# SreenivasVRao/SuperSloMo-VideoInterpolation-PyTorch

Hardware: AMD Instinct MI355X
Metric: interpolated 1280x720 frames/sec (higher is better)
Workload: dtype f32

## Files before the change

include/ssm_hip.h:

```cpp
#ifndef SSM_HIP_H
#define SSM_HIP_H

#include <stddef.h>

#ifdef __cplusplus
extern "C" {
#endif

#define SSM_PADX 4
#define SSM_PADY 3
#define SSM_TAIL_SLACK_FLOATS (1 << 16)

#define SSM_OK 0
#define SSM_E_ARG (-1)
#define SSM_E_LAUNCH (-2)
#define SSM_E_UNSUPPORTED (-3)

#define SSM_FLAG_LRELU 1
#define SSM_FLAG_FP16_FAST 2
#define SSM_FLAG_Q8 4
#define SSM_FLAG_MASK 8

typedef struct ssm_view {
    float *ptr;
    long long sb, sc;
    int sh;
} ssm_view;

typedef struct ssm_hview {
    void *ptr;
    long long sb, sg, sp;
    int sh;
} ssm_hview;

int ssm_abi_version(void);
const char *ssm_last_error_string(void);

void ssm_plane_dims(int H, int W, int *Hp, int *Wp);

int ssm_copy_view(ssm_view src, ssm_view dst, int B, int C, int H, int W, void *stream);

int ssm_conv_config(int k, int Cout, int B, int H, int W, int pool, int *BN, int *CK);
int ssm_conv_plan(int k, int Cin, int Cout, int B, int H, int W, int pool, int ups, int *kind, int *BN, int *CK);
int ssm_conv_force_kind(int kind);

size_t ssm_packed_weight_floats(int Cout, int Cin_padded, int k, int BN);
size_t ssm_packed_bias_floats(int Cout, int BN);

int ssm_pack_weights(const float *w_oihw, const float *bias, float *w_packed, float *bias_packed,
                     int Cout, int Cin, int Cin_padded, int k, int BN, void *stream);

int ssm_conv2d_fwd(ssm_view x1, int C1, ssm_view x2, int C2, const float *w_packed,
                   const float *bias_packed, ssm_view y, ssm_view pool, int B, int H, int W,
                   int Cout, int k, float slope, int flags, void *stream);

int ssm_conv2d_ups_fwd(ssm_view a, int C1, ssm_view b, int C2, const float *w_packed, const float *bias_packed,
                       ssm_view y, int B, int H, int W, int Cout, float slope, int flags, void *stream);

int ssm_conv2d_add_fwd(ssm_view x1, int C1, ssm_view x2, int C2, const float *w_packed, const float *bias_packed, ssm_view y,
                       ssm_view pool, ssm_view add, int add_div, int B, int H, int W, int Cout, int k, float slope, int flags,
                       void *stream);
int ssm_conv2d_ups_add_fwd(ssm_view a, int C1, ssm_view b, int C2, const float *w_packed, const float *bias_packed, ssm_view y,
                           ssm_view add, int add_div, int B, int H, int W, int Cout, float slope, int flags, void *stream);

int ssm_wino_plan(int Cin, int Cout, int B, int H, int W, int ups, int *kind, int *BN, int *CK);
int ssm_wino_force_kind(int kind);
size_t ssm_wino_packed_weight_floats(int Cout, int Cin, int BN);
int ssm_wino_pack_weights(const float *w_oihw, const float *bias, float *w_packed, float *bias_packed, int Cout, int Cin,
                          int BN, void *stream);
int ssm_wino_conv2d_fwd(ssm_view x1, int C1, ssm_view x2, int C2, const float *w_packed, const float *bias_packed,
                        ssm_view y, ssm_view pool, int B, int H, int W, int Cout, float slope, int flags, void *stream);
int ssm_wino_conv2d_ups_fwd(ssm_view a, int C1, ssm_view b, int C2, const float *w_packed, const float *bias_packed,
                            ssm_view y, int B, int H, int W, int Cout, float slope, int flags, void *stream);

int ssm_wino_splitk_plan(int Cin, int Cout, int B, int H, int W, int ups, int BN, int *KS);
int ssm_wino_conv2d_splitk_fwd(ssm_view x1, int C1, ssm_view x2, int C2, const float *w_packed, const float *bias_packed, ssm_view part,
                               int KS, int ups, int B, int H, int W, int Cout, int BN, void *stream);
int ssm_splitk_finish_fwd(ssm_view part, int KS, ssm_view y, ssm_view pool, ssm_view add, int add_div, int B, int C, int H, int W,
                          float slope, int flags, void *stream);
int ssm_conv_splitk_plan(int k, int Cin, int Cout, int B, int H, int W, int *KS);
int ssm_splitk_enable(int wino, int conv);
int ssm_conv2d_splitk_fwd(ssm_view x1, int C1, ssm_view x2, int C2, const float *w_packed, const float *bias_packed, ssm_view part,
                          int KS, int B, int H, int W, int Cout, int k, void *stream);
int ssm_wino_conv2d_add_fwd(ssm_view x1, int C1, ssm_view x2, int C2, const float *w_packed, const float *bias_packed, ssm_view y,
                            ssm_view pool, ssm_view add, int add_div, int B, int H, int W, int Cout, float slope, int flags,
                            void *stream);
int ssm_wino_conv2d_ups_add_fwd(ssm_view a, int C1, ssm_view b, int C2, const float *w_packed, const float *bias_packed, ssm_view y,
                                ssm_view add, int add_div, int B, int H, int W, int Cout, float slope, int flags, void *stream);

int ssm_wino4_plan(int Cin, int Cout, int B, int H, int W, int ups, int *kind, int *BN, int *CK);
int ssm_wino4_preferred(int Cin, int Cout, int B, int H, int W, int ups);
double ssm_wino_estimate(int Cin, int Cout, int B, int H, int W, int ups);
int ssm_wino4_force_kind(int kind);
size_t ssm_wino4_packed_weight_floats(int Cout, int Cin);
int ssm_wino4_pack_weights(const float *w_oihw, const float *bias, float *w_packed, float *bias_packed, int Cout, int Cin, void *stream);
int ssm_wino4_conv2d_add_fwd(ssm_view x1, int C1, ssm_view x2, int C2, const float *w_packed, const float *bias_packed, ssm_view y,
                             ssm_view pool, ssm_view add, int add_div, int B, int H, int W, int Cout, float slope, int flags,
                             void *stream);
int ssm_wino4_conv2d_ups_add_fwd(ssm_view a, int C1, ssm_view b, int C2, const float *w_packed, const float *bias_packed, ssm_view y,
                                 ssm_view add, int add_div, int B, int H, int W, int Cout, float slope, int flags, void *stream);
#define SSM_WINO4_BORDER_TH 16
#define SSM_WINO4_BORDER_TW 32
int ssm_wino4_conv2d_shuffle_fwd(ssm_view x1, int C1, ssm_view x2, int C2, const float *w_packed, const float *bias_packed, ssm_view y, int B,
                                 int H, int W, int Cout4, float slope, int flags, void *stream);
int ssm_wino4_conv2d_ups_border_fwd(ssm_view a, int C1, ssm_view b, int C2, const float *w_packed, const float *bias_packed, ssm_view y, int B,
                                    int H, int W, int Cout, float slope, int flags, void *stream);

int ssm_upgemm_supported(int Cin, int Cout, int H, int W, int k);
int ssm_upgemm_preferred(int Cin, int Cout, int B, int h, int w);
int ssm_upgemm_force_kind(int kind);
size_t ssm_upgemm_packed_weight_floats(int Cout, int Cin);
int ssm_upgemm_pack_weights(const float *w_oihw, float *w_packed, int Cout, int Cin, void *stream);
size_t ssm_upgemm_scratch_floats(int Cout, int B, int h, int w);
int ssm_upgemm_conv2d_ups_add_fwd(ssm_view a, int C1, ssm_view b, int C2, const float *w_packed, const float *bias, ssm_view scratch, ssm_view y,
                                  ssm_view add, int add_div, int B, int H, int W, int Cout, float slope, int flags, void *stream);

int ssm_wino1d_plan(int k, int Cin, int Cout, int B, int H, int W, int *kind, int *BN, int *CK);
int ssm_wino1d_force_kind(int kind);
size_t ssm_wino1d_packed_weight_floats(int Cout, int CinP, int k, int BN);
int ssm_wino1d_pack_weights(const float *w_oihw, const float *bias, float *w_packed, float *bias_packed, int Cout, int Cin,
                            int CinP, int k, int BN, void *stream);
int ssm_wino1d_conv2d_add_fwd(ssm_view x, int Cin, const float *w_packed, const float *bias_packed, ssm_view y, ssm_view pool,
                              ssm_view add, int add_div, int B, int H, int W, int Cout, int k, float slope, int flags, void *stream);

int ssm_wino7_plan(int Cin, int Cout, int B, int H, int W, int *kind);
int ssm_wino7_force_kind(int kind);
size_t ssm_wino7_packed_weight_floats(int Cout, int Cin);
int ssm_wino7_pack_weights(const float *w_oihw, const float *bias, float *w_packed, float *bias_packed, int Cout, int Cin, void *stream);
int ssm_wino7_conv2d_add_fwd(ssm_view x, int Cin, const float *w_packed, const float *bias_packed, ssm_view y, ssm_view pool,
                             ssm_view add, int add_div, int B, int H, int W, int Cout, float slope, int flags, void *stream);

int ssm_wino5_plan(int Cin, int Cout, int B, int H, int W, int *kind);
int ssm_wino5_force_kind(int kind);
size_t ssm_wino5_packed_weight_floats(int Cout, int CinP);
int ssm_wino5_pack_weights(const float *w_oihw, const float *bias, float *w_packed, float *bias_packed, int Cout, int Cin, int CinP,
                           void *stream);
int ssm_wino5_conv2d_add_fwd(ssm_view x, int Cin, const float *w_packed, const float *bias_packed, ssm_view y, ssm_view pool,
                             ssm_view add, int add_div, int B, int H, int W, int Cout, float slope, int flags, void *stream);

enum { SSM_PACK_DIRECT = 0, SSM_PACK_WINO = 1, SSM_PACK_WINO1D = 2, SSM_PACK_WINO4 = 3, SSM_PACK_WINO7 = 4, SSM_PACK_WINO5 = 5 };
typedef struct {
    const float *w;
    const float *bias;
    float *wp, *bp;
    int Cout, Cin, CinP, k, BN, algo, transposed, nbias;
    long long first, total;
} ssm_pack32_job;
int ssm_pack32_weights_batch(const ssm_pack32_job *jobs_device, int n_jobs, long long total_elements, void *stream);
int ssm_pack32_wino_tiles_batch(const ssm_pack32_job *jobs_device, int n_jobs, long long total_tiles, int max_bn, void *stream);

int ssm_conv16_config(int k, int Cout, int W, int *BN, int *KYS);
int ssm_conv16_plan(int k, int Cin, int Cout, int W, int ups, int flags, int *kind, int *BN, int *KYS);
size_t ssm_packed16_weight_halves(int Cout, int Cin_padded, int k, int BN);
int ssm_pack16_weights(const float *w_oihw, const float *bias, void *w_packed, float *bias_packed, int Cout,
                       int Cin, int Cin_padded, int k, int BN, int KYS, float scale, void *stream);
int ssm_conv2d_hl8_fwd(ssm_hview x1, int C1, ssm_hview x2, int C2, const void *w_packed,
                       const float *bias_packed, float wscale, ssm_hview y_hl8, ssm_view y_f32,
                       ssm_hview pool_hl8, int B, int H, int W, int Cout, int k, float slope, int flags,
                       void *stream);
int ssm_conv16_ups_config(int Cout, int W, int *BN, int *KYS);
int ssm_conv2d_ups_hl8_fwd(ssm_hview a, int C1, ssm_hview b, int C2, const void *w_packed,
                           const float *bias_packed, float wscale, ssm_hview y_hl8, ssm_view y_f32, int B, int H,
                           int W, int Cout, float slope, int flags, void *stream);
int ssm_conv16q_config(int k, int Cout, int W, int *BN, int *KYS);
int ssm_conv16q_ups_config(int Cout, int W, int *BN, int *KYS);
size_t ssm_packed16q_weight_bytes(int Cout, int Cin_padded, int k, int BN, int KYS);
int ssm_pack16q_weights(const float *w_oihw, const float *bias, void *w_packed, float *bias_packed, int Cout, int Cin,
                        int Cin_padded, int k, int BN, int KYS, float scale, void *stream);
int ssm_flowinterp_inputs_hq8_fwd(ssm_view img6, ssm_view flow4, const float *t, ssm_hview out16, ssm_view flows4, int B, int H,
                                  int W, void *stream);
int ssm_conv2d_hl8_subpixel_fwd(ssm_hview x1, int C1, ssm_hview x2, int C2, const void *w_packed, const float *bias_packed,
                                float inv_wscale, ssm_hview y_hl8, int B, int H, int W, int Cr, int transposed, float slope, int flags,
                                void *stream);
typedef struct ssm_subpixel_problem {
    ssm_hview x1;
    int C1;
    ssm_hview x2;
    int C2;
    const void *w_packed;
    const float *bias_packed;
    float inv_wscale;
    ssm_hview y_hl8;
    int H, W;
    int transposed;
    int skip_y, skip_x;
} ssm_subpixel_problem;
size_t ssm_conv16_subpixel_table_bytes(int n);
int ssm_conv16_subpixel_plan(const ssm_subpixel_problem *problems, int n, int B, int Cr, int wcfg, float slope, int flags,
                             void *table_host, size_t table_bytes, int *block_start);
int ssm_conv16_subpixel_run(const void *table_device, int n, const int *block_start, int Cr, int wcfg, int Cin, void *stream);
int ssm_hl8_gather_cols(ssm_hview a, int Ga, ssm_hview b, int Gb, ssm_hview dst, int B, int H, int col0, int ncols, int col1,
                        void *stream);
typedef struct ssm_pack16q_job {
    const float *w;
    const float *bias;
    void *wp;
    float *bp;
    int Cout, Cin, CinP, k, BN, KYS;
    float scale;
    int transposed;
    int block_start, row_blocks;
} ssm_pack16q_job;
int ssm_pack16q_job_blocks(int Cout, int CinP, int k, int BN, int *row_blocks, int *bias_blocks);
int ssm_pack16q_weights_batch(const ssm_pack16q_job *jobs_device, int n_jobs, int total_blocks, void *stream);
int ssm_hq8_from_f32(ssm_view src, ssm_hview dst, int B, int C, int G, int H, int W, void *stream);
int ssm_hq8_to_f32(ssm_hview src, ssm_view dst, int B, int C, int G, int H, int W, void *stream);
int ssm_hl8_from_f32(ssm_view src, ssm_hview dst, int B, int C, int G, int H, int W, void *stream);
int ssm_hl8_to_f32(ssm_hview src, ssm_view dst, int B, int C, int G, int H, int W, void *stream);

int ssm_upsample2x_cat_hl8_fwd(ssm_hview a, int Ga, ssm_hview b, int Gb, ssm_hview y, int B, int h, int w,
                               void *stream);
int ssm_flowinterp_inputs_hl8_fwd(ssm_view img6, ssm_view flow4, const float *t, ssm_hview out16,
                                  ssm_view flows4, int B, int H, int W, void *stream);

int ssm_avgpool2_fwd(ssm_view x, ssm_view y, int B, int C, int H, int W, void *stream);

int ssm_upsample2x_cat_fwd(ssm_view a, int Ca, ssm_view b, int Cb, ssm_view y, int B, int h, int w,
                           void *stream);

int ssm_warp_bilinear_fwd(ssm_view img, ssm_view flow, ssm_view out, int B, int C, int H, int W,
                          void *stream);

int ssm_flowinterp_inputs_fwd(ssm_view img6, ssm_view flow4, const float *t, ssm_view out16, int B,
                              int H, int W, void *stream);
int ssm_flowinterp_inputs_t_fwd(ssm_view img6, ssm_view flow4, const float *t, ssm_view out16, int B, int H, int W, void *stream);

int ssm_synthesize_fwd(ssm_view img6, ssm_view in16, ssm_view out5, const float *t, ssm_view y3,
                       ssm_view aux, int B, int H, int W, void *stream);

int ssm_synthesize_upscaled_fwd(ssm_view img6, ssm_view aux_lo, const float *t, ssm_view y3, int B, int H, int W, int s, void *stream);

int ssm_tile_stitch_fwd(ssm_view tile, ssm_view out, int N, int C, int window_h, int window_w, int Hp, int Wp, int oy, int ox, int cy0,
                        int cx0, int cy1, int cx1, int seams, int b, void *stream);

int ssm_final_conv_fwd(ssm_view x, const float *w_oihw, const float *bias, int NC, ssm_view out, ssm_view img6, ssm_view in16,
                       const float *t, ssm_view y3, ssm_view aux, int B, int H, int W, void *stream);

int ssm_program_create(void **handle);
int ssm_program_destroy(void *handle);
int ssm_program_begin(void *handle, void *const *streams, int n_streams);
int ssm_program_mark(void *handle, int *n_nodes);
int ssm_program_end(void *handle, int *n_nodes);
int ssm_program_run(void *handle, int first, int last, void *const *streams, int n_streams);
int ssm_stream_wait(void *src_stream, void *dst_stream);

int ssm_frames_from_u8_fwd(const unsigned char *frames_hwc, ssm_view out, int N, int H, int W, int Hp, int Wp,
                           int top, int left, const float *mean3, const float *std3, int pad_before_norm,
                           void *stream);
int ssm_frames_to_u8_fwd(ssm_view in, unsigned char *frames_hwc, int N, int H, int W, int top, int left,
                         const float *mean3, const float *std3, int mode, void *stream);

#define SSM_YUV_ROW 20
#define SSM_YUV_BT601 0
#define SSM_YUV_BT709 1
#define SSM_YUV_LIMITED 0
#define SSM_YUV_FULL 1
#define SSM_YUV_420_CENTRED 0
#define SSM_YUV_420_COSITED 1
#define SSM_YUV_444 2
// ... 154 lines not shown
```

superslomo-videointerpolation-pytorch_amd/csrc/ssm_wino4.hip:

```cpp
#include "ssm_conv_host.h"
#include "ssm_device.h"

#include <atomic>
#include <mutex>
#include <type_traits>
#include <cstdlib>

namespace {

struct W4Params {
    const float *src1;
    const float *src2;
    long long sb1, sb2;
    long long sc;
    int sh;
    int C1, Cin;
    const float *wpk;
    const float *bias;
    float *dst;
    long long dsb, dsc;
    int dsh;
    float *pool;
    long long psb, psc;
    int psh;
    int H, W, Cout;
    int hs, ws;
    int tilesX, tilesY, NB;
    float slope;
    int lrelu;
    int vec;
    int abl;
    unsigned long long *dbg;
    int trace_block;
    int stagger;
    int border;
    const float *add;
    long long asb, asc;
    int ash, adiv;
};

template <int GTX_, int WTY_, int WTX_, int NCB_ = 1>
struct W4Cfg {
    static constexpr int GTX = GTX_, GTY = 16 / GTX_, WTY = WTY_, WTX = WTX_, NCB = NCB_;
    static constexpr int NW = 4 * NCB, THREADS = 64 * NW;
    static constexpr int CK = 4, BN = 32 * NCB, NT = 32;
    static constexpr int NTX = GTX * WTX, NTY = GTY * WTY;
    static constexpr int TH = 4 * NTY, TW = 4 * NTX;
    static constexpr int PH = TH + 2, PW = TW + 8, PW4 = PW / 4;
    static constexpr int SHIFT = 1;
    static constexpr int USZ1 = CK * 9 * 32 * 4, USZ = NCB * USZ1;
    static constexpr int PSZ = CK * PH * PW;
    static constexpr int VSZ = CK * 9 * NT * 4;
    static constexpr int LH = TH / 2 + 2, LW = TW / 2 + 8, LW4 = LW / 4;
    static constexpr int RSZ = CK * LH * LW;
    static constexpr int NPOS = (TH / 2 + 1) * (TW / 2 + 1);
    static_assert(WTY * WTX == 2 && (GTX == 4 || GTX == 8 || GTX == 16) && (NCB == 1 || NCB == 2), "two tile groups of 16 tiles");
    static_assert(USZ1 % 256 == 0 && NPOS <= 256, "filter stage = whole 1-KiB DMA groups; expander: one position per thread");
};

template <class C, bool UPS>
struct W4Lds {
    static constexpr int DSZ = UPS ? C::RSZ : C::PSZ;
    static constexpr int DH = UPS ? C::LH : C::PH, DW4 = UPS ? C::LW4 : C::PW4;
    static constexpr int NGU = C::USZ / 256;
    static constexpr int NDQ = DSZ / 4;
    static constexpr int NGP = (NDQ + 63) / 64;
    static constexpr int NW = C::NCB == 2 ? 4 : C::NW;
    static constexpr int NIU = (NGU + NW - 1) / NW, NIP = (NGP + NW - 1) / NW, NI = NIU + NIP;
    static constexpr int NBUF = C::NCB == 2 ? 2 : 1;
    static constexpr int UOFF = 0;
    static constexpr int DOFF = 2 * C::USZ;
    static constexpr int DCAP = NGP * 256 + 256;
    static constexpr int NBD = 2;
    static constexpr int HOFF = DOFF + NBD * DCAP;
    static constexpr int HCAP = C::PSZ + 4;
    static constexpr int POFF = UPS ? HOFF : DOFF;
    static constexpr int PCAP = UPS ? HCAP : DCAP;
    static constexpr int VOFF = HOFF + (UPS ? NBUF * HCAP : 0);
    static constexpr int BYTES = (VOFF + NBUF * C::VSZ) * 4;
    static_assert(VOFF % 4 == 0 && DOFF % 4 == 0 && HOFF % 4 == 0 && HCAP % 4 == 0 && DCAP % 4 == 0, "16-byte aligned regions");
    static_assert(BYTES + (C::NCB == 2 ? 256 : 0) <= (C::NCB == 1 ? 80 : 160) * 1024, "LDS budget (two workgroups of 256 or one of 512 per CU; 64-cout form: + its biases)");
};

#define W4_PA 0.625
#define W4_PB 1.6
constexpr float kA = (float)W4_PA, kB = (float)W4_PB, kA2 = (float)(W4_PA * W4_PA), kB2 = (float)(W4_PB * W4_PB);
constexpr float kA3 = (float)(W4_PA * W4_PA * W4_PA), kB3 = (float)(W4_PB * W4_PB * W4_PB);
constexpr float kP0 = (float)(W4_PA * W4_PA * W4_PB * W4_PB), kS2 = (float)(W4_PA * W4_PA + W4_PB * W4_PB);

__host__ __device__ constexpr int w4_freq(int i, int j) { return 18 * (j / 3) + 3 * i + (j % 3); }

__device__ __forceinline__ void w4_row_pass(int hh, const float *d, float *x) {
    if (hh == 0) {
        const float te = d[4] - kB2 * d[2], to = d[3] - kB2 * d[1];
        x[0] = (kP0 * d[0] - kS2 * d[2]) + d[4];
        x[1] = te + kA * to;
        x[2] = te - kA * to;
    } else {
        const float ue = d[4] - kA2 * d[2], uo = d[3] - kA2 * d[1];
        x[0] = ue + kB * uo;
        x[1] = ue - kB * uo;
        x[2] = (kP0 * d[1] - kS2 * d[3]) + d[5];
    }
}

__device__ __forceinline__ void w4_col_pass(float x0, float x1, float x2, float x3, float x4, float x5, float *v, int stride) {
    const float te = x4 - kB2 * x2, to = x3 - kB2 * x1;
    const float ue = x4 - kA2 * x2, uo = x3 - kA2 * x1;
    v[0] = (kP0 * x0 - kS2 * x2) + x4;
    v[stride] = te + kA * to;
    v[2 * stride] = te - kA * to;
    v[3 * stride] = ue + kB * uo;
    v[4 * stride] = ue - kB * uo;
    v[5 * stride] = (kP0 * x1 - kS2 * x3) + x5;
}

__device__ __forceinline__ void w4_col_pass_half(int hq, float x0, float x1, float x2, float x3, float x4, float x5, float *v, int stride) {
    if (hq == 0) {
        const float te = x4 - kB2 * x2, to = x3 - kB2 * x1;
        v[0] = (kP0 * x0 - kS2 * x2) + x4;
        v[stride] = te + kA * to;
        v[2 * stride] = te - kA * to;
    } else {
        const float ue = x4 - kA2 * x2, uo = x3 - kA2 * x1;
        v[0] = ue + kB * uo;
        v[stride] = ue - kB * uo;
        v[2 * stride] = (kP0 * x1 - kS2 * x3) + x5;
    }
}

template <int NT>
__device__ __forceinline__ void w4_store_v9(int part, const float *v, f32x4 *vo) {
    float *vf = (float *)vo;
    if (part == 0) {
        vo[0] = f32x4{v[0], v[1], v[2], v[3]};
        vo[NT] = f32x4{v[4], v[5], v[6], v[7]};
        vf[2 * NT * 4] = v[8];
    } else if (part == 1) {
        vf[2 * NT * 4 + 1] = v[0];
        *(f32x2 *)(vf + 2 * NT * 4 + 2) = f32x2{v[1], v[2]};
        vo[3 * NT] = f32x4{v[3], v[4], v[5], v[6]};
        *(f32x2 *)(vf + 4 * NT * 4) = f32x2{v[7], v[8]};
    } else if (part == 2) {
        *(f32x2 *)(vf + 4 * NT * 4 + 2) = f32x2{v[0], v[1]};
        vo[5 * NT] = f32x4{v[2], v[3], v[4], v[5]};
        *(f32x2 *)(vf + 6 * NT * 4) = f32x2{v[6], v[7]};
        vf[6 * NT * 4 + 2] = v[8];
    } else {
        vf[6 * NT * 4 + 3] = v[0];
        vo[7 * NT] = f32x4{v[1], v[2], v[3], v[4]};
        vo[8 * NT] = f32x4{v[5], v[6], v[7], v[8]};
    }
}

template <int NT>
__device__ __forceinline__ void w4_store_v(int hh, const float *v, f32x4 *vo) {
    if (hh == 0) {
#pragma unroll
        for (int g = 0; g < 4; ++g) vo[g * NT] = f32x4{v[4 * g], v[4 * g + 1], v[4 * g + 2], v[4 * g + 3]};
        *(f32x2 *)(vo + 4 * NT) = f32x2{v[16], v[17]};
    } else {
        *((f32x2 *)(vo + 4 * NT) + 1) = f32x2{v[0], v[1]};
#pragma unroll
        for (int g = 0; g < 4; ++g) vo[(5 + g) * NT] = f32x4{v[2 + 4 * g], v[3 + 4 * g], v[4 + 4 * g], v[5 + 4 * g]};
    }
}

#ifdef SSM_WINO_ABLATE
#define W4ABL(bit) (p.abl & (bit))
#elif defined(W4_CT_ABL)
#define W4ABL(bit) (W4_CT_ABL & (bit))
#else
#define W4ABL(bit) 0
#endif

template <bool SHUF>
__device__ __forceinline__ void w4_epilogue_shuffle(const W4Params &p, const f32x4 (&acc)[36], const float (&bv)[4], int b, int cu0, int q, int px, int py);

__device__ __forceinline__ void w4_epilogue(const W4Params &p, const f32x4 (&acc)[36], const float (&bv)[4], int b, int cu0, int q, int px, int py) {
        const float sl = (p.lrelu & 1) ? p.slope : 1.f;
        const bool amask = (p.lrelu & 2) != 0;
        float *dstb = p.dst + (long long)b * p.dsb;
        float *poolb = p.pool ? p.pool + (long long)b * p.psb : nullptr;
                const unsigned pb = 4u * ((unsigned)(4 * q) * (unsigned)p.dsc + (unsigned)py * (unsigned)p.dsh + (unsigned)px);
        const unsigned qb = 4u * ((unsigned)(4 * q) * (unsigned)p.psc + (unsigned)(py >> 1) * (unsigned)p.psh + (unsigned)(px >> 1));
        const bool vok = py + 4 <= p.H && px + 4 <= p.W && p.vec;
        const float *addb = p.add ? p.add + (long long)(b / p.adiv) * p.asb + (long long)(4 * q) * p.asc + (long long)py * p.ash + px : nullptr;
#pragma unroll
        for (int r = 0; r < 4; ++r) {
            const int cu = cu0 + r;
            float t[4][6];
#pragma unroll
            for (int j = 0; j < 6; ++j) {
                const float m0 = acc[w4_freq(0, j)][r], m1 = acc[w4_freq(1, j)][r], m2 = acc[w4_freq(2, j)][r], m3 = acc[w4_freq(3, j)][r],
                            m4 = acc[w4_freq(4, j)][r], m5 = acc[w4_freq(5, j)][r];
                const float s1 = m1 + m2, d1 = m1 - m2, s2 = m3 + m4, d2 = m3 - m4;
                t[0][j] = (m0 + s1) + s2;
                t[1][j] = kA * d1 + kB * d2;
                t[2][j] = kA2 * s1 + kB2 * s2;
                t[3][j] = (kA3 * d1 + m5) + kB3 * d2;
            }
            float y[4][4];
#pragma unroll
            for (int i = 0; i < 4; ++i) {
                const float s1 = t[i][1] + t[i][2], d1 = t[i][1] - t[i][2], s2 = t[i][3] + t[i][4], d2 = t[i][3] - t[i][4];
                y[i][0] = ((t[i][0] + s1) + s2) + bv[r];
                y[i][1] = (kA * d1 + kB * d2) + bv[r];
                y[i][2] = (kA2 * s1 + kB2 * s2) + bv[r];
                y[i][3] = ((kA3 * d1 + t[i][5]) + kB3 * d2) + bv[r];
            }
            if (addb) {
                const float *ap = addb + (long long)cu * p.asc;
#pragma unroll
                for (int i = 0; i < 4; ++i) {
                    if (vok) {
                        const f32x4 z = *(const f32x4 *)(ap + (long long)i * p.ash);
                        if (amask) {
#pragma unroll
                            for (int e = 0; e < 4; ++e) y[i][e] *= z[e] > 0.f ? 1.f : p.slope;
                        } else {
                            y[i][0] += z[0];
                            y[i][1] += z[1];
                            y[i][2] += z[2];
                            y[i][3] += z[3];
                        }
                    } else {
#pragma unroll
                        for (int e = 0; e < 4; ++e)
                            if (py + i < p.H && px + e < p.W) {
                                const float z = ap[(long long)i * p.ash + e];
                                if (amask) y[i][e] *= z > 0.f ? 1.f : p.slope;
                                else y[i][e] += z;
                            }
                    }
                }
            }
#pragma unroll
            for (int i = 0; i < 4; ++i)
#pragma unroll
                for (int e = 0; e < 4; ++e) y[i][e] = fmaxf(y[i][e], y[i][e] * sl);
            float *bp = dstb + (long long)cu * p.dsc;
#pragma unroll
            for (int i = 0; i < 4; ++i) {
                if (vok) {
                    store_sbase(bp + (long long)i * p.dsh, pb, f32x4{y[i][0], y[i][1], y[i][2], y[i][3]});
                } else {
#pragma unroll
                    for (int e = 0; e < 4; ++e)
                        if (py + i < p.H && px + e < p.W) store_sbase(bp + (long long)i * p.dsh + e, pb, y[i][e]);
                }
            }
            if (poolb) {
                float *qp = poolb + (long long)cu * p.psc;
#pragma unroll
                for (int i = 0; i < 2; ++i) {
                    const float o0 = ((y[2 * i][0] + y[2 * i + 1][0]) + (y[2 * i][1] + y[2 * i + 1][1])) * 0.25f;
                    const float o1 = ((y[2 * i][2] + y[2 * i + 1][2]) + (y[2 * i][3] + y[2 * i + 1][3])) * 0.25f;
                    const bool rok = py + 2 * i < p.H;
                    if (rok && px + 4 <= p.W && p.vec) store_sbase(qp + (long long)i * p.psh, qb, f32x2{o0, o1});
                    else if (rok) {
                        if (px + 2 <= p.W) store_sbase(qp + (long long)i * p.psh, qb, o0);
                        if (px + 4 <= p.W) store_sbase(qp + (long long)i * p.psh + 1, qb, o1);
                    }
                }
            }
            __builtin_amdgcn_sched_barrier(0);
        }
}

__device__ __forceinline__ void w4_output_tile(const f32x4 (&acc)[36], int r, float bias, float sl, float (&y)[4][4]) {
    float t[4][6];
#pragma unroll
    for (int j = 0; j < 6; ++j) {
        const float m0 = acc[w4_freq(0, j)][r], m1 = acc[w4_freq(1, j)][r], m2 = acc[w4_freq(2, j)][r], m3 = acc[w4_freq(3, j)][r],
                    m4 = acc[w4_freq(4, j)][r], m5 = acc[w4_freq(5, j)][r];
        const float s1 = m1 + m2, d1 = m1 - m2, s2 = m3 + m4, d2 = m3 - m4;
        t[0][j] = (m0 + s1) + s2;
        t[1][j] = kA * d1 + kB * d2;
        t[2][j] = kA2 * s1 + kB2 * s2;
        t[3][j] = (kA3 * d1 + m5) + kB3 * d2;
    }
#pragma unroll
    for (int i = 0; i < 4; ++i) {
        const float s1 = t[i][1] + t[i][2], d1 = t[i][1] - t[i][2], s2 = t[i][3] + t[i][4], d2 = t[i][3] - t[i][4];
        y[i][0] = ((t[i][0] + s1) + s2) + bias;
        y[i][1] = (kA * d1 + kB * d2) + bias;
        y[i][2] = (kA2 * s1 + kB2 * s2) + bias;
        y[i][3] = ((kA3 * d1 + t[i][5]) + kB3 * d2) + bias;
    }
#pragma unroll
    for (int i = 0; i < 4; ++i)
#pragma unroll
        for (int e = 0; e < 4; ++e) y[i][e] = fmaxf(y[i][e], y[i][e] * sl);
}

template <>
__device__ __forceinline__ void w4_epilogue_shuffle<true>(const W4Params &p, const f32x4 (&acc)[36], const float (&bv)[4], int b, int cu0, int q, int px, int py) {
    const float sl = (p.lrelu & 1) ? p.slope : 1.f;
    float *dstb = p.dst + (long long)b * p.dsb + (long long)(cu0 >> 2) * p.dsc;
    const unsigned pb = 4u * ((unsigned)q * (unsigned)p.dsc + (unsigned)(2 * py) * (unsigned)p.dsh + (unsigned)(2 * px));
    const bool vok = py + 4 <= p.H && px + 4 <= p.W && p.vec;
#pragma unroll
    for (int a = 0; a < 2; ++a) {
        float y0[4][4], y1[4][4];
        w4_output_tile(acc, 2 * a, bv[2 * a], sl, y0);
        w4_output_tile(acc, 2 * a + 1, bv[2 * a + 1], sl, y1);
#pragma unroll
        for (int i = 0; i < 4; ++i) {
            const float *rowp = dstb + (long long)(2 * i + a) * p.dsh;
            if (vok) {
                store_sbase_nop(rowp, pb, f32x4{y0[i][0], y1[i][0], y0[i][1], y1[i][1]});
                store_sbase_nop(rowp + 4, pb, f32x4{y0[i][2], y1[i][2], y0[i][3], y1[i][3]});
            } else {
#pragma unroll
                for (int e = 0; e < 4; ++e) {
                    if (py + i < p.H && px + e < p.W) {
                        store_sbase(rowp + 2 * e, pb, y0[i][e]);
                        store_sbase(rowp + 2 * e + 1, pb, y1[i][e]);
                    }
                }
            }
        }
        __builtin_amdgcn_sched_barrier(0);
    }
}

template <class C, bool UPS, bool SHUF = false>
__global__ __launch_bounds__(C::THREADS, 2) void wino4_kernel(const W4Params p) {
    extern __shared__ __attribute__((aligned(16))) float lds[];
    using L = W4Lds<C, UPS>;
    constexpr int BN = C::BN, PH = C::PH, PW = C::PW, CK = C::CK, NT = C::NT, NW = C::NW, NCB = C::NCB;

    const int tid = threadIdx.x;
    const int lane = tid & 63, l15 = lane & 15, q = lane >> 4;
    const int wid = __builtin_amdgcn_readfirstlane(tid >> 6);
    const int cb = wid & 1, tg = (wid >> 1) & 1, blk = wid >> 2;

    int id = ssm_xcd_tile(blockIdx.x, gridDim.x);
    const int nb = id % p.NB;
    id /= p.NB;
    int tx, ty, b;
    if (UPS && C::NCB == 1 && p.border) {
        const int nbt = 2 * p.tilesX + 2 * (p.tilesY - 2);
        const int k = id % nbt;
        b = id / nbt;
        if (k < 2 * p.tilesX) {
            ty = k < p.tilesX ? 0 : p.tilesY - 1;
            tx = k < p.tilesX ? k : k - p.tilesX;
        } else {
            const int kk = k - 2 * p.tilesX;
            ty = 1 + (kk >> 1);
            tx = (kk & 1) ? p.tilesX - 1 : 0;
        }
    } else {
        tx = id % p.tilesX;
        id /= p.tilesX;
        ty = id % p.tilesY;
        b = id / p.tilesY;
    }
    const int x0 = tx * C::TW, y0 = ty * C::TH;

    const long long porg = UPS ? (long long)(y0 / 2 - 1) * p.sh + (x0 / 2 - 4) : (long long)(y0 - 1) * p.sh + (x0 - 4);
    const float *pbase1 = p.src1 + (long long)b * p.sb1 + porg;
    const float *pbase2 = p.src2 + (long long)b * p.sb2 + porg;
    const float *wbase = p.wpk + (long long)nb * NCB * p.Cin * (9 * 32 * 4);

    int poff[L::NIP];
#pragma unroll
    for (int i = 0; i < L::NIP; ++i) {
        const int qq = (i * L::NW + (wid & (L::NW - 1))) * 64 + lane;
        if (qq < L::NDQ) {
            const int c = qq / (L::DH * L::DW4);
            const int rem = qq - c * (L::DH * L::DW4);
            const int r = rem / L::DW4;
            const int j = rem - r * L::DW4;
            const int sH = UPS ? p.hs : p.H, sW = UPS ? p.ws : p.W, sy = UPS ? y0 / 2 - 1 : y0 - 1, sx = UPS ? x0 / 2 : x0;
            const int re = min(r, sH + (SSM_PADY - 1) - sy), fe = min(4 * j, ((sW + 2 * SSM_PADX + 3) & ~3) - 4 - sx);
            poff[i] = ((int)(c * p.sc) + re * p.sh + fe) * 4;
        } else {
            poff[i] = 0;
        }
    }
    const int uoff = lane * 16;
    int uoffk[L::NIU];
#pragma unroll
    for (int k = 0; k < L::NIU; ++k) uoffk[k] = lane * 16 + k * (L::NW * 1024);
    const unsigned lds0 = (unsigned)(size_t)(__attribute__((address_space(3))) void *)lds;

    auto issue_k = [&](int ch, int stage, int k, int pbuf = 0) {
        constexpr int NW = L::NW;
        if (NCB == 2 && wid >= NW) return;
        const int c0 = ch * CK;
        if (k < L::NIU) {
            const int g = NW * k + wid;
            if (NW * k + NW - 1 < L::NGU || g < L::NGU) {
                constexpr int G1 = C::USZ1 / 256;
                const int gb = NCB == 1 ? 0 : g / G1;
                const float *base = wbase + ((long long)gb * p.Cin + c0) * (9 * 32 * 4) + (g - gb * G1) * 256;
                const unsigned m0v = __builtin_amdgcn_readfirstlane(lds0 + (unsigned)(L::UOFF + stage * C::USZ) * 4u + (unsigned)g * 1024u);
                lds_dma16(base, uoff, m0v);
            }
        } else {
            const int kk = k - L::NIU;
            const int g = NW * kk + wid;
            if (NW * kk + NW - 1 < L::NGP || g < L::NGP) {
                const float *base = (c0 < p.C1) ? pbase1 + (long long)c0 * p.sc : pbase2 + (long long)(c0 - p.C1) * p.sc;
                const unsigned m0v = __builtin_amdgcn_readfirstlane(lds0 + (unsigned)(L::DOFF + pbuf * L::DCAP) * 4u + (unsigned)g * 1024u + (UPS ? 0u : 4u * C::SHIFT));
                lds_dma16(base, poff[kk], m0v);
            }
        }
    };

    f32x4 acc[36];
#pragma unroll
    for (int f = 0; f < 36; ++f) acc[f] = f32x4{0.f, 0.f, 0.f, 0.f};

    const int nchunks = p.Cin / CK;
    if (p.stagger > 0 && ((blockIdx.x >> 8) & 1)) {
        for (int i = 0; i < p.stagger; ++i) __builtin_amdgcn_s_sleep(1);
    }
    static_assert(L::NI <= (NCB == 2 ? 18 : 9), "DMA issue slots of the matrix loop: one per frequency group (two in the 512-thread form)");
    auto issue_n = [&](int ch, int stage, int n) { issue_k(ch, stage, n < L::NIP ? L::NIU + n : n - L::NIP); };
    const bool u_full = wid < L::NGU - NW * (L::NIU - 1);
    if constexpr (NCB == 1) {
#pragma unroll
        for (int n = 0; n < L::NI; ++n) issue_n(0, 0, n);
        if (p.Cin / CK > 1) {
#pragma unroll
            for (int k = L::NIU; k < L::NI; ++k) issue_k(1, 0, k, 1);
        }
    }
    float bv[4];
    if constexpr (NCB == 2) {
        if (tid < BN) lds[L::BYTES / 4 + tid] = p.bias[nb * BN + tid];
    } else {
#pragma unroll
        for (int r = 0; r < 4; ++r) bv[r] = p.bias[nb * BN + blk * 32 + cb * 16 + 4 * q + r];
    }

    const int thh = (wid >> 1) & 1;
    const int thq = wid >> 2;
    const int tu = tid & 127;
    const int tcin = tu >> 5, ttile = tu & 31;
    const int tgx = (ttile & 15) % C::GTX, tgy = (ttile & 15) / C::GTX, tg2 = ttile >> 4;
    const int tTx = (tg2 % C::WTX) * C::GTX + tgx, tTy = (tg2 / C::WTX) * C::GTY + tgy;
    const int t_src = L::POFF + (UPS ? 0 : C::SHIFT) + (tcin * PH + 4 * tTy) * PW + 4 * tTx + 3 + (UPS ? C::SHIFT : 0);
    const int t_dst = L::VOFF / 4 + (tcin * 9) * NT + ttile;

    const f32x4 *lds4 = (const f32x4 *)lds;
    const int aBase = L::UOFF / 4 + blk * (C::USZ1 / 4) + q * (9 * 32) + cb * 16 + l15;
    const int bBase = L::VOFF / 4 + q * (9 * NT) + tg * 16 + l15;

    int ex_r0 = 0, ex_r1 = 0, ex_dd = 0, ex_fl = 0;
    if constexpr (UPS) {
        constexpr int PRW = C::TW / 2 + 1, NPOS = C::NPOS, LW = C::LW;
        const int etid = threadIdx.x & 255;
        const int ly0 = y0 / 2 - 1, lx0 = x0 / 2 - 1;
        const int pi = etid / PRW, pj = etid - pi * PRW;
        const int i = ly0 + pi, j = lx0 + pj;
        const int i0 = min(max(i, 0), p.hs - 1), i1 = min(max(i + 1, 0), p.hs - 1);
        const int j0 = min(max(j, 0), p.ws - 1), j1 = min(max(j + 1, 0), p.ws - 1);
        const int Y = 2 * i + 1, X = 2 * j + 1;
        const bool yt = Y >= 0 && Y < p.H, yb2 = Y + 1 < p.H, xl = X >= 0 && X < p.W, xr = X + 1 < p.W;
        ex_fl = (j0 == j1 ? 1 : 0) | (i0 == i1 ? 2 : 0) | ((yt && xl) ? 4 : 0) | ((yt && xr) ? 8 : 0) | ((yb2 && xl) ? 16 : 0) | ((yb2 && xr) ? 32 : 0) |
                (etid < NPOS ? 64 : 0);
        ex_r0 = (i0 - ly0) * LW + 3 - lx0 + j0;
        ex_r1 = (i1 - ly0) * LW + 3 - lx0 + j0;
        ex_dd = (2 * pi) * PW + 2 * pj + 3 + C::SHIFT;
    }
    auto expand = [&](int rbuf, int hbuf, auto CB, auto CN) {
        if constexpr (UPS) {
            constexpr int LH = C::LH, LW = C::LW;
            constexpr int cbeg = decltype(CB)::value, cnum = decltype(CN)::value;
            const float *raw = lds + L::DOFF + rbuf * L::DCAP + cbeg * LH * LW;
            float *hip = lds + L::HOFF + hbuf * L::HCAP + cbeg * PH * PW;
            if (ex_fl & 64) {
                const bool jeq = ex_fl & 1, ieq = ex_fl & 2;
                const float ex_xa = jeq ? 1.f : 0.75f, ex_xb = jeq ? 0.f : 0.25f;
                const float ex_ca = jeq ? 1.f : 0.25f, ex_cw = jeq ? 0.f : 0.75f;
                const float ya = ieq ? 1.f : 0.75f, yb = ieq ? 0.f : 0.25f;
                const float ex_a00 = (ex_fl & 4) ? ya : 0.f, ex_b00 = (ex_fl & 4) ? yb : 0.f;
                const float ex_a01 = (ex_fl & 8) ? ya : 0.f, ex_b01 = (ex_fl & 8) ? yb : 0.f;
                const float ex_a10 = (ex_fl & 16) ? yb : 0.f, ex_b10 = (ex_fl & 16) ? ya : 0.f;
                const float ex_a11 = (ex_fl & 32) ? yb : 0.f, ex_b11 = (ex_fl & 32) ? ya : 0.f;
                const float *r0 = raw + ex_r0, *r1 = raw + ex_r1;
                float *dd = hip + ex_dd;
                float v00[cnum], v01[cnum], v10[cnum], v11[cnum];
#pragma unroll
                for (int cc = 0; cc < cnum; ++cc) {
                    v00[cc] = r0[cc * LH * LW];
                    v01[cc] = r0[cc * LH * LW + 1];
                    v10[cc] = r1[cc * LH * LW];
                    v11[cc] = r1[cc * LH * LW + 1];
                }
#pragma unroll
                for (int cc = 0; cc < cnum; ++cc) {
                    const float h00 = ex_xa * v00[cc] + ex_xb * v01[cc], h01 = ex_ca * v00[cc] + ex_cw * v01[cc];
                    const float h10 = ex_xa * v10[cc] + ex_xb * v11[cc], h11 = ex_ca * v10[cc] + ex_cw * v11[cc];
                    dd[cc * PH * PW] = ex_a00 * h00 + ex_b00 * h10;
                    dd[cc * PH * PW + 1] = ex_a01 * h01 + ex_b01 * h11;
                    dd[cc * PH * PW + PW] = ex_a10 * h00 + ex_b10 * h10;
                    dd[cc * PH * PW + PW + 1] = ex_a11 * h01 + ex_b11 * h11;
                }
            }
        }
    };

    auto transform_as = [&](auto HH, auto HQ, int sbuf, int vbuf) {
        constexpr int hh = decltype(HH)::value, hq = decltype(HQ)::value;
        const float *rp = lds + t_src + sbuf * L::PCAP;
        f32x4 *vo = (f32x4 *)lds + t_dst + vbuf * (C::VSZ / 4);
        f32x4 a4[6];
        f32x2 a2[6];
#pragma unroll
        for (int i = 0; i < 6; ++i) {
            a4[i] = *(const f32x4 *)(rp + i * PW);
            a2[i] = *(const f32x2 *)(rp + i * PW + 4);
        }
        float X[6][3];
#pragma unroll
        for (int i = 0; i < 6; ++i) {
            const float d[6] = {a4[i][0], a4[i][1], a4[i][2], a4[i][3], a2[i][0], a2[i][1]};
            w4_row_pass(hh, d, X[i]);
        }
        if constexpr (NCB == 1) {
            float v[18];
#pragma unroll
            for (int jj = 0; jj < 3; ++jj) w4_col_pass(X[0][jj], X[1][jj], X[2][jj], X[3][jj], X[4][jj], X[5][jj], v + jj, 3);
            w4_store_v<NT>(hh, v, vo);
        } else {
            float v[9];
#pragma unroll
            for (int jj = 0; jj < 3; ++jj) w4_col_pass_half(hq, X[0][jj], X[1][jj], X[2][jj], X[3][jj], X[4][jj], X[5][jj], v + jj, 3);
            w4_store_v9<NT>(2 * hh + hq, v, vo);
        }
    };
    auto transform = [&](int sbuf = 0, int vbuf = 0) {
        using I0 = std::integral_constant<int, 0>;
        using I1 = std::integral_constant<int, 1>;
        if constexpr (NCB == 1) {
            if (thh == 0) transform_as(I0{}, I0{}, sbuf, vbuf);
            else transform_as(I1{}, I0{}, sbuf, vbuf);
        } else {
            if (thh == 0) {
                if (thq == 0) transform_as(I0{}, I0{}, sbuf, vbuf);
                else transform_as(I0{}, I1{}, sbuf, vbuf);
            } else {
                if (thq == 0) transform_as(I1{}, I0{}, sbuf, vbuf);
                else transform_as(I1{}, I1{}, sbuf, vbuf);
            }
        }
    };

#ifdef SSM_WINO_ABLATE
    unsigned long long tph[5] = {0, 0, 0, 0, 0};
    const bool stamp = (p.abl & 32) && p.dbg;
    unsigned long long tk = stamp ? __builtin_amdgcn_s_memtime() : 0;
    const unsigned long long tstart = tk;
#define W4STAMP(i)                                              \
    if (stamp) {                                                \
        const unsigned long long tn = __builtin_amdgcn_s_memtime(); \
        tph[i] += tn - tk;                                      \
        tk = tn;                                                \
    }
    const bool trace = (p.abl & 128) && p.dbg && blockIdx.x == 0;
#define W4TRACE(chv, pt)                                                                                             \
    if (trace && (chv) < 16 && lane == 0) p.dbg[16 + (wid * 16 + (chv)) * 4 + (pt)] = __builtin_amdgcn_s_memtime();
#elif defined(W4_TRACE)
#define W4STAMP(i)
    unsigned long long *ltrace = (unsigned long long *)(lds + L::BYTES / 4 + 64);
    const bool trace = p.dbg && blockIdx.x == (unsigned)p.trace_block;
#define W4TRACE(chv, pt) \
    if (trace && (chv) < 16 && lane == 0) ltrace[(wid * 16 + (chv)) * 4 + (pt)] = __builtin_amdgcn_s_memtime();
    if (trace && lane == 0) ltrace[(wid * 16 + 0) * 4 + 1] = __builtin_amdgcn_s_memtime();
#else
#define W4STAMP(i)
#define W4TRACE(chv, pt)
#endif
    f32x4 a[3], bq[3];
    auto matrix = [&](int stage, int vbuf, auto dma, auto slot) __attribute__((always_inline)) {
        const int ai = aBase + stage * (C::USZ / 4), bi = bBase + vbuf * (C::VSZ / 4);
        a[0] = lds4[ai];
        bq[0] = lds4[bi];
        a[1] = lds4[ai + 32];
        bq[1] = lds4[bi + NT];
#pragma unroll
        for (int g = 0; g < 9; ++g) {
            const int cur = g % 3, nxt = (g + 2) % 3;
#pragma unroll
            for (int e = 0; e < 4; ++e) {
                acc[4 * g + e] = __builtin_amdgcn_mfma_f32_16x16x4f32(a[cur][e], bq[cur][e], acc[4 * g + e], 0, 0, 0);
                if (e == 0) {
                    __builtin_amdgcn_sched_barrier(0);
                    if (g + 2 < 9 && !W4ABL(8)) {
                        a[nxt] = lds4[ai + (g + 2) * 32];
                        bq[nxt] = lds4[bi + (g + 2) * NT];
                    }
                    __builtin_amdgcn_sched_barrier(0);
                }
                if constexpr (NCB == 2) {
                    slot(4 * g + e);
                    __builtin_amdgcn_sched_barrier(0);
                }
                if constexpr (NCB == 2) {
                    if ((e == 1 || e == 3) && 2 * g + (e == 3) < L::NI) {
                        dma(2 * g + (e == 3));
                        __builtin_amdgcn_sched_barrier(0);
                    }
                } else if (e == 1 && g < L::NI) {
                    dma(g);
                    __builtin_amdgcn_sched_barrier(0);
                }
            }
            __builtin_amdgcn_sched_barrier(0);
        }
    };

    if constexpr (NCB == 1) {
        static_assert(L::NGP % L::NW == 0, "every wave brings NIP patch pieces per chunk");
        auto chunk1 = [&](int ch, auto N1, auto N2) __attribute__((always_inline)) {
            constexpr bool n1 = decltype(N1)::value, n2 = decltype(N2)::value;
            const int stage = ch & 1;
            if (u_full) wait_vmcnt<L::NIU + (n1 ? L::NIP : 0)>();
            else wait_vmcnt<L::NIU - 1 + (n1 ? L::NIP : 0)>();
            __syncthreads();
            W4STAMP(0)
            if constexpr (UPS) {
                expand(stage, 0, std::integral_constant<int, 0>{}, std::integral_constant<int, CK>{});
                __syncthreads();
            }
            if (!W4ABL(4) || ch == 0) transform(UPS ? 0 : stage, 0);
            W4STAMP(1)
            wait_vmcnt<n1 ? L::NIP : 0>();
            __syncthreads();
            W4STAMP(2)
            const int (&uk)[L::NIU] = uoffk;
            const int (&pk)[L::NIP] = poff;
            const int c1 = (ch + 1) * CK, c2 = (ch + 2) * CK;
            const float *fb = wbase + wid * 256 + (long long)c1 * (9 * 32 * 4);
            const float *pb = (c2 < p.C1) ? pbase1 + (long long)c2 * p.sc : pbase2 + (long long)(c2 - p.C1) * p.sc;
            const unsigned mu = __builtin_amdgcn_readfirstlane(lds0 + (unsigned)(L::UOFF + (stage ^ 1) * C::USZ) * 4u + (unsigned)wid * 1024u);
            const unsigned mp = __builtin_amdgcn_readfirstlane(lds0 + (unsigned)(L::DOFF + stage * L::DCAP) * 4u + (unsigned)wid * 1024u + (UPS ? 0u : 4u * C::SHIFT));
            matrix(stage, 0, [&](int n) {
                if (W4ABL(1) && ch >= 1) return;
                constexpr int NW = L::NW;
                if (n < L::NIU) {
                    if constexpr (n1) {
                        if (NW * n + NW - 1 < L::NGU || NW * n + wid < L::NGU)
                            lds_dma16(fb, uk[n], mu + (unsigned)(n * NW * 1024));
                    }
                } else if constexpr (n2) {
                    const int k = n - L::NIU;
                    lds_dma16(pb, pk[k], mp + (unsigned)(k * NW * 1024));
                }
            }, [](int) {});
            W4STAMP(3)
        };
        using T = std::true_type;
        using F = std::false_type;
        int ch = 0;
        for (; ch + 2 < nchunks; ++ch) chunk1(ch, T{}, T{});
        if (ch + 1 < nchunks) chunk1(ch++, T{}, F{});
        chunk1(ch, F{}, F{});

    } else {
        using T = std::true_type;
        using F = std::false_type;
#pragma unroll
        for (int k = 0; k < L::NI; ++k) issue_k(0, 0, k, 0);
        if (nchunks > 1) {
#pragma unroll
            for (int k = L::NIU; k < L::NI; ++k) issue_k(1, 0, k, 1);
        }
        wait_vmcnt<0>();
        __syncthreads();
        using C0 = std::integral_constant<int, 0>;
        using C2 = std::integral_constant<int, 2>;
        auto expand_half = [&](int rbuf, int hbuf) {
            if (blk == 0) expand(rbuf, hbuf, C0{}, C2{});
            else expand(rbuf, hbuf, C2{}, C2{});
        };
        if constexpr (UPS) {
            expand_half(0, 0);
            if (nchunks > 1) expand_half(1, 1);
            __syncthreads();
            if (nchunks > 2) {
#pragma unroll
                for (int k = L::NIU; k < L::NI; ++k) issue_k(2, 0, k, 0);
            }
        }
        transform(0, 0);
        f32x4 r4[6];
        f32x2 r2[6];
        float tX[6][3];
        float tv18[18];
        auto tstep2 = [&](auto HH, int m, const float *src, f32x4 *vo) __attribute__((always_inline)) {
            constexpr int hh = decltype(HH)::value;
            if (m < 6) {
                r4[m] = *(const f32x4 *)(src + m * PW);
                r2[m] = *(const f32x2 *)(src + m * PW + 4);
            }
            if (m >= 3 && m < 9) {
                const int i = m - 3;
                const float d[6] = {r4[i][0], r4[i][1], r4[i][2], r4[i][3], r2[i][0], r2[i][1]};
                w4_row_pass(hh, d, tX[i]);
            }
            if (m >= 9 && m < 18) {
                const int jj = (m - 9) / 3, st3 = (m - 9) % 3;
                const float x0v = tX[0][jj], x1v = tX[1][jj], x2v = tX[2][jj], x3v = tX[3][jj], x4v = tX[4][jj], x5v = tX[5][jj];
                if (st3 == 0) {
                    tv18[jj] = (kP0 * x0v - kS2 * x2v) + x4v;
                    tv18[15 + jj] = (kP0 * x1v - kS2 * x3v) + x5v;
                }
                if (st3 == 1) {
                    const float te = x4v - kB2 * x2v, to = x3v - kB2 * x1v;
                    tv18[3 + jj] = te + kA * to;
                    tv18[6 + jj] = te - kA * to;
                }
                if (st3 == 2) {
                    const float ue = x4v - kA2 * x2v, uo = x3v - kA2 * x1v;
                    tv18[9 + jj] = ue + kB * uo;
                    tv18[12 + jj] = ue - kB * uo;
                }
            }
            if (m >= 18 && m < 23) {
                const int k = m - 18;
                if (hh == 0) {
                    if (k < 4) vo[k * NT] = f32x4{tv18[4 * k], tv18[4 * k + 1], tv18[4 * k + 2], tv18[4 * k + 3]};
                    else *(f32x2 *)(vo + 4 * NT) = f32x2{tv18[16], tv18[17]};
                } else {
                    if (k == 0) *((f32x2 *)(vo + 4 * NT) + 1) = f32x2{tv18[0], tv18[1]};
                    else vo[(4 + k) * NT] = f32x4{tv18[4 * k - 2], tv18[4 * k - 1], tv18[4 * k], tv18[4 * k + 1]};
                }
            }
        };
        auto chunk = [&](int ch, auto STEADY, auto HH, auto HQ) __attribute__((always_inline)) {
            constexpr bool steady = decltype(STEADY)::value;
            const bool m1 = steady || ch + 1 < nchunks, m2 = steady || ch + 2 < nchunks, m3 = steady || ch + 3 < nchunks;
            const int st = ch & 1;
            wait_vmcnt<0>();
            if (!W4ABL(16) || ch == 0) __syncthreads();
            W4STAMP(0)
            W4TRACE(ch, 0)
            const float *tsrc = lds + t_src + (st ^ 1) * L::PCAP;
            f32x4 *tdst = (f32x4 *)lds + t_dst + (st ^ 1) * (C::VSZ / 4);
            matrix(st, st, [&](int g) {
                if (W4ABL(1) || decltype(HQ)::value != 0) return;
                if (g < L::NIU) {
                    if (m1) issue_k(ch + 1, st ^ 1, g, 0);
                } else if constexpr (UPS) {
                    if (m3) issue_k(ch + 3, 0, g, st ^ 1);
                } else {
                    if (m2) issue_k(ch + 2, 0, g, st);
                }
            }, [&](int m) {
                if constexpr (decltype(HQ)::value == 1) {
                    if (m1 && !W4ABL(4)) tstep2(HH, m, tsrc, tdst);
                }
            });
            W4STAMP(3)
            W4TRACE(ch, 2)
            if constexpr (UPS) {
                if (m2 && decltype(HQ)::value == 0) expand(st, st, C0{}, std::integral_constant<int, CK>{});
            }
            W4STAMP(1)
            W4TRACE(ch, 3)
        };
        auto chunks = [&](auto HH, auto HQ) __attribute__((always_inline)) {
            if constexpr (decltype(HQ)::value == 1) __builtin_amdgcn_s_setprio(1);
            int ch = 0;
            for (; ch + 3 < nchunks; ++ch) chunk(ch, T{}, HH, HQ);
            for (; ch < nchunks; ++ch) chunk(ch, F{}, HH, HQ);
        };
        using I0 = std::integral_constant<int, 0>;
        using I1 = std::integral_constant<int, 1>;
        if (thh == 0) {
            if (thq == 0) chunks(I0{}, I0{});
            else chunks(I0{}, I1{});
        } else {
            if (thq == 0) chunks(I1{}, I0{});
            else chunks(I1{}, I1{});
        }
    }

#if defined(SSM_WINO_ABLATE) || defined(W4_CT_ABL)
    if (W4ABL(2) && acc[0][0] != 12345.678f) return;
#endif
    {
        if constexpr (NCB == 2) {
            const f32x4 b4 = *(const f32x4 *)(lds + L::BYTES / 4 + blk * 32 + cb * 16 + 4 * q);
            bv[0] = b4[0], bv[1] = b4[1], bv[2] = b4[2], bv[3] = b4[3];
        }
        const int gx = l15 % C::GTX, gy = l15 / C::GTX;
        const int Tx = (tg % C::WTX) * C::GTX + gx, Ty = (tg / C::WTX) * C::GTY + gy;
        if constexpr (SHUF) w4_epilogue_shuffle<true>(p, acc, bv, b, nb * BN + blk * 32 + cb * 16, q, x0 + 4 * Tx, y0 + 4 * Ty);
        else w4_epilogue(p, acc, bv, b, nb * BN + blk * 32 + cb * 16, q, x0 + 4 * Tx, y0 + 4 * Ty);
    }
#if defined(W4_TRACE) && !defined(SSM_WINO_ABLATE)
    if (trace) {
        if (lane == 0) ltrace[(wid * 16 + 1) * 4 + 1] = __builtin_amdgcn_s_memtime();
        wait_vmcnt<0>();
        if (lane == 0) ltrace[(wid * 16 + 2) * 4 + 1] = __builtin_amdgcn_s_memtime();
        __syncthreads();
        for (int i = tid; i < NW * 64; i += C::THREADS) p.dbg[16 + i] = ltrace[i];
    }
#endif
#ifdef SSM_WINO_ABLATE
    if (stamp) {
        wait_vmcnt<0>();
        W4STAMP(4)
        if (tid == 0) {
            for (int i = 0; i < 5; ++i) atomicAdd(p.dbg + i, tph[i]);
            atomicAdd(p.dbg + 5, tk - tstart);
            atomicAdd(p.dbg + 6, 1ULL);
        }
    }
#endif
}

using X4A = W4Cfg<8, 2, 1>;
using X4B = W4Cfg<16, 2, 1>;
using X4C = W4Cfg<4, 1, 2>;

using Y4A = W4Cfg<8, 2, 1, 2>;
using Y4B = W4Cfg<16, 2, 1, 2>;
using Y4C = W4Cfg<4, 1, 2, 2>;


#define SSM_W4_KINDS(X) X(X4A_, X4A) X(X4B_, X4B) X(X4C_, X4C) X(Y4A_, Y4A) X(Y4B_, Y4B) X(Y4C_, Y4C)

enum W4Kind {
#define X(name, cfg) name,
    SSM_W4_KINDS(X)
#undef X
        NW4KIND
};

struct W4KindInfo {
    int th, tw, bn;
};

constexpr W4KindInfo kW4Info[NW4KIND] = {
#define X(name, cfg) W4KindInfo{cfg::TH, cfg::TW, cfg::BN},
    SSM_W4_KINDS(X)
#undef X
};

ssm::ForcedKind g_force_w4kind;
constexpr ssm::OutRules kW4Rules = { true,  4,  false};
#if defined(SSM_WINO_ABLATE) || defined(W4_TRACE)
std::atomic<unsigned long long *> g_w4dbg{nullptr};
#endif

double estimate_w4(const W4KindInfo &ki, int Cin, int Cout, int B, int H, int W, int ups) {
    const long long tiles = (long long)B * ((W + ki.tw - 1) / ki.tw) * ((H + ki.th - 1) / ki.th);
    const long long nwg = tiles * (Cout / ki.bn);
    const double chunks = (double)Cin / 4.0;
    if (ki.bn == 64) {
        const double per = chunks * 3500.0 + 24000.0;
        return (double)((nwg + 255) / 256) * per;
    }
    const double per = chunks * (4500.0 + (ups ? 250.0 : 0.0)) + 11000.0;
    const long long full = nwg / 512, rem = nwg % 512;
    double t = (double)full * per;
    if (rem) t += rem > 256 ? per : chunks * (3300.0 + (ups ? 250.0 : 0.0)) + 11000.0;
    return t;
}

int pick_w4kind(int Cin, int Cout, int B, int H, int W, int ups) {
    const int forced = g_force_w4kind.get(NW4KIND);
    if (forced >= 0) return forced;
    int best = -1;
    double bt = 0.0;
    static const int allow_wide = [] {
        const char *e = getenv("SSM_WINO4_WIDE");
        return e ? atoi(e) : 1;
    }();
    for (int i = 0; i < NW4KIND; ++i) {
        if (kW4Info[i].bn == 64 && (!allow_wide || Cout % 64)) continue;
        const double t = estimate_w4(kW4Info[i], Cin, Cout, B, H, W, ups);
        if (best < 0 || t < bt * 0.999) {
            best = i;
            bt = t;
        }
    }
    return best;
}

template <class C, bool UPS, bool SHUF = false>
int w4launch(W4Params &p, int B, hipStream_t st) {
    p.tilesX = (p.W + C::TW - 1) / C::TW;
    p.tilesY = (p.H + C::TH - 1) / C::TH;
    if (p.Cout % C::BN) {
        ssm::set_error("wino4 conv: tile configuration of %d couts per workgroup, Cout = %d", C::BN, p.Cout);
        return SSM_E_UNSUPPORTED;
    }
    p.NB = p.Cout / C::BN;
    if (p.border && (!UPS || p.tilesX < 2 || p.tilesY < 2)) {
        ssm::set_error("wino4 conv: a border-ring launch needs the fused-upsample form and at least 2 x 2 workgroup tiles (%d x %d)", p.tilesX, p.tilesY);
        return SSM_E_UNSUPPORTED;
    }
    const long long ntiles = p.border ? 2LL * p.tilesX + 2LL * (p.tilesY - 2) : (long long)p.tilesX * p.tilesY;
    const long long blocks = ntiles * p.NB * B;
    int lds_bytes = W4Lds<C, UPS>::BYTES + (C::NCB == 2 ? C::BN * 4 : 0);
#ifdef W4_TRACE
    lds_bytes += 4096;
#endif
#ifdef SSM_WINO_ABLATE
    if (const char *e = getenv("SSM_WINO4_SOLO"))
        if (atoi(e) && lds_bytes < 100 * 1024) lds_bytes = 100 * 1024;
#endif
    return ssm::launch_tiles<wino4_kernel<C, UPS, SHUF>>("wino4 conv", UPS ? "ssm_wino4_conv2d_ups_fwd" : "ssm_wino4_conv2d_fwd", blocks, C::THREADS,
                                                          lds_bytes, st, p);
}

template <bool UPS>
int w4dispatch(int kind, W4Params &p, int B, hipStream_t st) {
    switch (kind) {
#define X(name, cfg) \
    case name: return w4launch<cfg, UPS>(p, B, st);
        SSM_W4_KINDS(X)
#undef X
    }
    ssm::set_error("wino4 conv: tile configuration %d is not available for this problem", kind);
    return SSM_E_UNSUPPORTED;
}

__global__ void wino4_pack_kernel(const float *__restrict__ w, const float *__restrict__ bias, float *__restrict__ wp,
                                  float *__restrict__ bp, int Cout, int Cin, long long total, int nbias) {
    const long long idx = (long long)blockIdx.x * blockDim.x + threadIdx.x;
    if (idx < total) {
        long long r = idx;
        const int e = (int)(r % 4);
        r /= 4;
        const int n = (int)(r % 32);
        r /= 32;
        const int fq = (int)(r % 9);
        r /= 9;
        const int cin = (int)(r % Cin);
        const int nb = (int)(r / Cin);
        const int co = nb * 32 + n, f = 4 * fq + e, i = (f % 18) / 3, j = 3 * (f / 18) + f % 3;
        double val = 0.0;
        if (co < Cout) {
            auto grow = [](int f, double (&g)[3]) {
                const double p = f == 0 ? 0.0 : f == 1 ? W4_PA : f == 2 ? -W4_PA : f == 3 ? W4_PB : -W4_PB;
                if (f == 5) {
                    g[0] = g[1] = 0.0;
                    g[2] = 1.0;
                    return;
                }
                double nrm = 1.0;
#pragma unroll
                for (int o = 0; o < 5; ++o) {
                    const double po = o == 0 ? 0.0 : o == 1 ? W4_PA : o == 2 ? -W4_PA : o == 3 ? W4_PB : -W4_PB;
                    if (o != f) nrm *= p - po;
                }
                g[0] = 1.0 / nrm;
                g[1] = p / nrm;
                g[2] = p * p / nrm;
            };
            double gi[3], gj[3];
            grow(i, gi);
            grow(j, gj);
            const float *g = w + ((long long)co * Cin + cin) * 9;
#pragma unroll
            for (int a = 0; a < 3; ++a)
#pragma unroll
                for (int c = 0; c < 3; ++c) val += gi[a] * (double)g[3 * a + c] * gj[c];
        }
        wp[idx] = (float)val;
    }
    if (idx < nbias) bp[idx] = (idx < Cout) ? bias[idx] : 0.f;
}

int w4fill(W4Params &p, ssm_view x1, int C1, ssm_view x2, int C2, const float *w_packed, const float *bias_packed, ssm_view y, ssm_view pool,
           ssm_view add, int add_div, int B, int H, int W, int Cout, float slope, int flags, int srcW) {
    SSM_REQUIRE(B > 0 && H > 0 && W > 0 && Cout > 0 && C1 > 0 && C2 >= 0, "wino4 conv: bad sizes");
    SSM_REQUIRE(Cout % 32 == 0, "wino4 conv: Cout (%d) must be a multiple of 32", Cout);
    SSM_REQUIRE(x1.ptr && y.ptr && w_packed && bias_packed, "wino4 conv: null pointer");
    SSM_REQUIRE(C1 % 4 == 0 && C2 % 4 == 0, "wino4 conv: channel counts (%d,%d) must be multiples of 4", C1, C2);
    SSM_TRY(ssm::check_source("wino4 conv", true, x1, srcW, w_packed));
    SSM_TRY(ssm::check_source2("wino4 conv", x1, x2, C2));
    SSM_REQUIRE(4LL * x1.sc * 4 < 0x7fffffffLL, "wino4 conv: channel stride too large");
    p.src1 = x1.ptr;
    p.src2 = C2 > 0 ? x2.ptr : x1.ptr;
    p.sb1 = x1.sb;
    p.sb2 = C2 > 0 ? x2.sb : 0;
    p.sc = x1.sc;
    p.sh = x1.sh;
    p.C1 = C1;
    p.Cin = C1 + C2;
    p.wpk = w_packed;
    p.bias = bias_packed;
    p.hs = H / 2;
    p.ws = W / 2;
    p.abl = 0;
    p.border = 0;
#ifdef SSM_WINO_ABLATE
    if (const char *e = getenv("SSM_WINO4_ABL")) p.abl = atoi(e);
#endif
#if defined(SSM_WINO_ABLATE) || defined(W4_TRACE)
    p.dbg = g_w4dbg.load();
#else
    p.dbg = nullptr;
#endif
    static const int stagger = [] {
        const char *e = getenv("SSM_WINO4_STAGGER");
        return e ? atoi(e) : 0;
    }();
    p.stagger = stagger;
    p.trace_block = 0;
#ifdef W4_TRACE
    if (const char *e = getenv("SSM_W4_TRACE_BLOCK")) p.trace_block = atoi(e);
#endif
    return ssm::bind_outputs("wino4 conv", kW4Rules, p, y, pool, add, add_div, B, H, W, Cout, slope, flags);
}

}

extern "C" int ssm_wino4_plan(int Cin, int Cout, int B, int H, int W, int ups, int *kind, int *BN, int *CK) {
    if (Cin % 4 || Cout % 32 || Cin <= 0 || Cout <= 0) {
        ssm::set_error("wino4 conv: no tile configuration for Cin=%d Cout=%d (Cin a multiple of 4, Cout a multiple of 32)", Cin, Cout);
        return SSM_E_UNSUPPORTED;
    }
    if (kind) *kind = pick_w4kind(Cin, Cout, B, H, W, ups);
    if (BN) *BN = 32;
    if (CK) *CK = 4;
    return SSM_OK;
}

#if defined(SSM_WINO_ABLATE) || defined(W4_TRACE)
extern "C" int ssm_wino4_debug_buffer(unsigned long long *dev_counters) {
    g_w4dbg.store(dev_counters);
    return SSM_OK;
}
#endif

extern "C" int ssm_wino4_preferred(int Cin, int Cout, int B, int H, int W, int ups) {
    if (Cin % 4 || Cout % 32 || Cin <= 0 || Cout <= 0) return 0;
    if ((long long)H * W < 2048) return 0;
    return 1;
}

extern "C" int ssm_wino4_force_kind(int kind) {
    return g_force_w4kind.set(kind, NW4KIND);
}

extern "C" size_t ssm_wino4_packed_weight_floats(int Cout, int Cin) { return (size_t)(Cout / 32) * (size_t)Cin * 9 * 32 * 4; }

extern "C" int ssm_wino4_pack_weights(const float *w, const float *bias, float *wp, float *bp, int Cout, int Cin, void *stream) {
    SSM_REQUIRE(w && bias && wp && bp, "wino4 pack_weights: null pointer");
    SSM_REQUIRE(Cout > 0 && Cin > 0 && Cout % 32 == 0, "wino4 pack_weights: bad sizes (Cout a multiple of 32)");
    const long long total = (long long)ssm_wino4_packed_weight_floats(Cout, Cin);
    const int nbias = Cout;
    const long long n = total > nbias ? total : nbias;
    SSM_LAUNCH(wino4_pack_kernel, dim3((unsigned)((n + 255) / 256)), dim3(256), 0, (hipStream_t)stream, w, bias, wp, bp, Cout, Cin,
                       total, nbias);
    return ssm::check_launch("ssm_wino4_pack_weights");
}

extern "C" int ssm_wino4_conv2d_add_fwd(ssm_view x1, int C1, ssm_view x2, int C2, const float *w_packed, const float *bias_packed, ssm_view y,
                                        ssm_view pool, ssm_view add, int add_div, int B, int H, int W, int Cout, float slope, int flags,
                                        void *stream) {
    int kind = 0;
    const int rc = ssm_wino4_plan(C1 + C2, Cout, B, H, W, 0, &kind, nullptr, nullptr);
    if (rc != SSM_OK) return rc;
    W4Params p;
    const int rf = w4fill(p, x1, C1, x2, C2, w_packed, bias_packed, y, pool, add, add_div, B, H, W, Cout, slope, flags, W);
    if (rf != SSM_OK) return rf;
    return w4dispatch<false>(kind, p, B, (hipStream_t)stream);
}

extern "C" int ssm_wino4_conv2d_shuffle_fwd(ssm_view x1, int C1, ssm_view x2, int C2, const float *w_packed, const float *bias_packed, ssm_view y,
                                            int B, int H, int W, int Cout4, float slope, int flags, void *stream) {
    SSM_REQUIRE(Cout4 > 0 && Cout4 % 64 == 0, "wino4 conv_shuffle: 4 Cout (%d) must be a multiple of 64", Cout4);
    int kind = 0;
    const int rc = ssm_wino4_plan(C1 + C2, Cout4, B, H, W, 0, &kind, nullptr, nullptr);
    if (rc != SSM_OK) return rc;
    if (kW4Info[kind].bn != 64) kind = Y4A_;
    W4Params p;
    const ssm_view none = {nullptr, 0, 0, 0};
    const int rf = w4fill(p, x1, C1, x2, C2, w_packed, bias_packed, y, none, none, 1, B, H, W, Cout4, slope, flags, W);
    if (rf != SSM_OK) return rf;
    switch (kind) {
        case Y4A_: return w4launch<Y4A, false, true>(p, B, (hipStream_t)stream);
        case Y4B_: return w4launch<Y4B, false, true>(p, B, (hipStream_t)stream);
        default: return w4launch<Y4C, false, true>(p, B, (hipStream_t)stream);
    }
}

extern "C" int ssm_wino4_conv2d_ups_border_fwd(ssm_view a, int C1, ssm_view b, int C2, const float *w_packed, const float *bias_packed, ssm_view y,
                                               int B, int H, int W, int Cout, float slope, int flags, void *stream) {
    SSM_REQUIRE(H % 2 == 0 && W % 2 == 0, "wino4 conv_ups_border: the output of a x2 upsample has even H, W (got %dx%d)", H, W);
    SSM_REQUIRE(C1 + C2 > 0 && (C1 + C2) % 4 == 0 && Cout % 32 == 0, "wino4 conv_ups_border: Cin a multiple of 4, Cout of 32");
    W4Params p;
    const ssm_view none = {nullptr, 0, 0, 0};
    const int rf = w4fill(p, a, C1, b, C2, w_packed, bias_packed, y, none, none, 1, B, H, W, Cout, slope, flags, W / 2);
    if (rf != SSM_OK) return rf;
    p.border = 1;
    return w4launch<X4A, true>(p, B, (hipStream_t)stream);
}

extern "C" int ssm_wino4_conv2d_ups_add_fwd(ssm_view a, int C1, ssm_view b, int C2, const float *w_packed, const float *bias_packed, ssm_view y,
                                            ssm_view add, int add_div, int B, int H, int W, int Cout, float slope, int flags, void *stream) {
    int kind = 0;
    SSM_REQUIRE(H % 2 == 0 && W % 2 == 0, "wino4 conv_ups: the output of a x2 upsample has even H, W (got %dx%d)", H, W);
    const int rc = ssm_wino4_plan(C1 + C2, Cout, B, H, W, 1, &kind, nullptr, nullptr);
    if (rc != SSM_OK) return rc;
    W4Params p;
    const ssm_view none = {nullptr, 0, 0, 0};
    const int rf = w4fill(p, a, C1, b, C2, w_packed, bias_packed, y, none, add, add_div, B, H, W, Cout, slope, flags, W / 2);
    if (rf != SSM_OK) return rf;
    return w4dispatch<true>(kind, p, B, (hipStream_t)stream);
}
```

superslomo-videointerpolation-pytorch_amd/ssm_amd/engine.py:

```python
import os

import torch

from . import hipbind as hb
from .weights import RECURRENT_HIDDEN, RECURRENT_LAYERS, param_key, recurrent_convs, unet_layers


class KernelTimer:

    def __init__(self):
        self.spans = []

    def span(self, family, name, flops=0.0, nbytes=0.0, issued=None):
        e0, e1 = torch.cuda.Event(enable_timing=True), torch.cuda.Event(enable_timing=True)
        self.spans.append((family, name, flops, nbytes, e0, e1, flops if issued is None else issued))
        return e0, e1

    def summary(self):
        out = {}
        for fam, name, fl, nb, e0, e1, isd in self.spans:
            d = out.setdefault(fam, {"ms": 0.0, "flops": 0.0, "issued": 0.0, "bytes": 0.0, "launches": 0, "by_name": {}})
            ms = e0.elapsed_time(e1)
            d["ms"] += ms
            d["flops"] += fl
            d["issued"] += isd
            d["bytes"] += nb
            d["launches"] += 1
            n = d["by_name"].setdefault(name, [0.0, 0.0, 0])
            n[0] += ms
            n[1] += fl
            n[2] += 1
        return out


MODES = ("f32", "f32w", "f16x3", "f16", "f16f8")


def base_mode(mode):
    return "f32" if mode == "f32w" else mode


HOIST_PAIR_PARTS = os.environ.get("SSM_HOIST", "1") != "0"

WINO_SKIP = frozenset(n for n in os.environ.get("SSM_WINO_SKIP", "").split(",") if n)

WINO1D = os.environ.get("SSM_WINO1D", "57")


WINO7 = os.environ.get("SSM_WINO7", "1")
WINO5 = os.environ.get("SSM_WINO5", "1")


WINO4 = os.environ.get("SSM_WINO4", "1")


TRAIN_WINO4 = os.environ.get("SSM_TRAIN_WINO4", "1")
TRAIN_FWD_BLOCKED = os.environ.get("SSM_TRAIN_FWD_BLOCKED", "1")


WINO4_SUBPIXEL = tuple(n for n in os.environ.get("SSM_WINO4_SUBPIXEL", "conv11a").split(",") if n not in ("", "0"))


UPGEMM = os.environ.get("SSM_UPGEMM", "1")


def upgemm_enabled(name):
    return UPGEMM not in ("0", "") and (UPGEMM == "1" or name in UPGEMM.split(","))


def wino4_enabled(name):
    return WINO4 not in ("0", "") and (WINO4 == "1" or name in WINO4.split(","))


def wino1d_enabled(k):
    return k in (5, 7) and str(k) in WINO1D


def choose_algo(name, ci, co, k, nb, h, w, ups, wino, wino1d, wino4=None, blocked2d=None, upgemm=True):
    skip = name in WINO_SKIP or "all" in WINO_SKIP or name == "final_conv"
    wino4 = wino1d if wino4 is None else wino4
    blocked2d = wino1d if blocked2d is None else blocked2d
    if (upgemm and wino and wino1d and ups and not skip and k == 3 and upgemm_enabled(name) and hb.upgemm_supported(ci, co, h, w, k)
            and (UPGEMM != "1" or hb.upgemm_preferred(ci, co, nb, h, w))):
        return "upgemm"
    if blocked2d and not skip and k == 7 and WINO7 not in ("0", "") and hb.wino7_supported(ci, co, h, w, k):
        return "wino7"
    if blocked2d and not skip and k == 5 and WINO5 not in ("0", "") and ci % 4 == 0 and hb.wino5_supported(ci, co, h, w, k):
        return "wino5"
    if wino1d and not skip and wino1d_enabled(k) and hb.wino1d_supported(ci, co, h, w, k):
        return "wino1d"
    if wino and not skip and hb.wino_supported(ci, co, h, w, k):
        if (wino4 and wino4_enabled(name) and hb.wino4_supported(ci, co, h, w, k)
                and (WINO4 != "1" or hb.wino4_preferred(ci, co, nb, h, w, ups))):
            return "wino4"
        return "wino"
    return "direct"


_ALGO_CLASS = {name: (lambda form=form: form.cls) for name, form in hb.FORMS.items()}
ISSUED_FACTOR = {name: form.issued for name, form in hb.FORMS.items()}


def issued_factor(pk):
    return ISSUED_FACTOR.get(getattr(pk, "algo", "direct"), ISSUED_FACTOR["direct"])(pk.k)


def conv_fn(pk, ups=False):
    form = hb.FORMS[pk.algo]
    assert ups or form.launch is not None, "the low-res GEMM form is for the fused-upsample layers"
    return form.launch_ups if ups and form.launch_ups is not None else form.launch


POOLED = ("conv1b", "conv2b", "conv3b", "conv4b", "conv5b")
_SCALE = (("conv10", 2), ("conv11", 1), ("conv1", 1), ("conv2", 2), ("conv3", 4), ("conv4", 8), ("conv5", 16),
          ("conv6", 32), ("conv7", 16), ("conv8", 8), ("conv9", 4), ("fuse_conv", 1), ("final_conv", 1))


def layer_scale(name):
    for prefix, s in _SCALE:
        if name.startswith(prefix):
            return s
    raise KeyError(name)


class UNetPlan:
    timer = None
    RESCALE_EVERY = int(os.environ.get("SSM_RESCALE_EVERY", "256"))
    fast_layers = frozenset()

    DECODER = ("conv7a", "conv7b", "conv8a", "conv8b", "conv9a", "conv9b", "conv10a", "conv10b", "conv11a", "conv11b",
               "fuse_conv", "final_conv")
    ENCODER_T = ("c1", "c2", "c3", "c4", "c5", "c6")
    UPS = ("conv7a", "conv8a", "conv9a", "conv10a", "conv11a")

    CONV_OUT = ("t1a", "c1", "t2a", "c2", "t3a", "c3", "t4a", "c4", "t5a", "c5", "t6a", "c6", "t7a", "c7", "t8a", "c8", "t9a", "c9",
                "t10a", "c10", "t11a", "c11", "tf")

    def __init__(self, stage, state_dict, B, H, W, device, cross_skip=True, mode="f32", fuse_upsample=True,
                 bottleneck="CONV", seq_len=1, dec=None, twins=False, final4=None, hoist=None):
        assert mode in MODES, "precision mode must be one of %s" % (MODES,)
        self.wino = mode == "f32w"
        self.mode_name, mode = mode, base_mode(mode)
        assert bottleneck in ("CONV", "CLSTM", "CGRU"), "Unknown bottleneck type: %s" % bottleneck
        assert B % seq_len == 0
        self.bottleneck = bottleneck
        self.twins = bool(twins) and mode != "f32"
        self.scales = {}
        self.dec_b0, self.Bd = dec if dec is not None else (0, B)
        assert 0 <= self.dec_b0 and self.dec_b0 + self.Bd <= B
        self._b0 = 0
        self._Bcur = B
        self.mode, self.hl8, self.q8 = mode, mode != "f32", mode == "f16f8"
        self.fuse_up = bool(fuse_upsample)
        infer_plan = self.fuse_up and not twins
        self.wino1d = self.wino and infer_plan
        self.blocked2d = self.wino and (infer_plan or TRAIN_FWD_BLOCKED == "1")
        self.wino4 = self.wino and (infer_plan or TRAIN_WINO4 == "1")
        self.hoist = None
        self._pair_parts_ready = False
        if hoist is not None and stage == 2 and mode == "f32" and self.fuse_up and not twins and hoist[1] > 1 and bottleneck == "CONV":
            assert B == hoist[0] * hoist[1] and dec is None
            self.hoist = (int(hoist[0]), int(hoist[1]))
        self.final4 = (mode == "f32" and self.fuse_up) if final4 is None else (bool(final4) and mode == "f32")
        if self.q8:
            assert self.fuse_up, "mode f16f8 covers the plan with the concat+upsample fused into the convolutions"
        if H % 32 or W % 32:
            raise AssertionError("H and W must be multiples of 32 (got %dx%d): the U-Net pools 5 times "
                                 "and concatenates skips (unchecked in the reference, fails in torch.cat)" % (H, W))
        self.stage, self.B, self.H, self.W, self.device = stage, B, H, W, device
        self.cross = bool(cross_skip) and stage == 2
        self.layers = {n: (ci, co, k) for n, ci, co, k in unet_layers(stage, cross_skip, bottleneck)}
        self.pk = {}
        self.refresh_weights(state_dict, check_shapes=True)
        self.rnn = None
        if bottleneck != "CONV":
            self.rnn = RecurrentBottleneck(bottleneck, state_dict, B // seq_len, seq_len, H // 32, W // 32, device, self.mode_name)
        Bd = self.Bd
        if self.hl8:
            P = lambda c, s: hb.HPlanes(B, c, H // s, W // s, device, q8=self.q8)
            D = lambda c, s: hb.HPlanes(Bd, c, H // s, W // s, device, q8=self.q8)
        else:
            P = lambda c, s: hb.Planes(B, c, H // s, W // s, device)
            D = lambda c, s: hb.Planes(Bd, c, H // s, W // s, device)
        cin0 = self.layers["conv1a"][0]
        cfin = self.layers["final_conv"][1]
        t = self.t = {}
        t["in"] = hb.HPlanes(B, cin0, H, W, device, groups=self.pk["conv1a"].cin_p // 8, q8=self.q8) if self.hl8 else P(cin0, 1)
        t["t1a"], t["c1"], t["p2"] = P(32, 1), P(32, 1), P(32, 2)
        t["t2a"], t["c2"], t["p3"] = P(64, 2), P(64, 2), P(64, 4)
        t["t3a"], t["c3"], t["p4"] = P(128, 4), P(128, 4), P(128, 8)
        t["t4a"], t["c4"], t["p5"] = P(256, 8), P(256, 8), P(256, 16)
        t["t5a"], t["c5"], t["p6"] = P(512, 16), P(512, 16), P(512, 32)
        t["c6"] = P(512, 32)
        if bottleneck == "CONV":
            t["t6a"] = P(512, 32)
        if not self.fuse_up:
            t["u7"] = D(1024 if self.cross else 512, 16)
            t["u8"], t["u9"], t["u10"], t["u11"] = D(1024, 8), D(512, 4), D(256, 2), D(128, 1)
        t["t7a"], t["c7"] = D(512, 16), D(512, 16)
        t["t8a"], t["c8"] = D(256, 8), D(256, 8)
        t["t9a"], t["c9"] = D(128, 4), D(128, 4)
        t["t10a"], t["c10"] = D(64, 2), D(64, 2)
        t["t11a"], t["c11"] = D(32, 1), D(32, 1)
        t["tf"] = D(32, 1)
        t["out"] = hb.Planes(Bd, cfin, H, W, device)
        if self.hoist:
            t["pair1a"] = hb.Planes(self.hoist[0], 32, H, W, device)
            if self.cross:
                t["pair7a"] = hb.Planes(self.hoist[0], 512, H // 16, W // 16, device)
        self.f32 = {}
        if self.twins:
            assert bottleneck == "CONV" and dec is None, "fp32 twins are for the training plan"
            for name in self.CONV_OUT + ("in",):
                ref = t[name]
                self.f32[name] = hb.Planes(B, ref.C if name != "in" else cin0, ref.H, ref.W, device)

    def refresh_weights(self, state_dict, check_shapes=False):
        self.sp, self._sd_for_sp = {}, state_dict
        self.pk_pair = {}
        tensors = []
        for name in self.layers:
            tensors += [state_dict[param_key(name, "weight")], state_dict[param_key(name, "bias")]]
        batchable = self.q8 and all(t.is_cuda and t.dtype == torch.float32 and t.is_contiguous() for t in tensors)
        self._refreshes = getattr(self, "_refreshes", 0) + 1
        if self._refreshes % self.RESCALE_EVERY == 0:
            self.scales, self._pack = {}, None
        if batchable and getattr(self, "_pack", None) is not None and self._pack[0] == hb.PackBatch.key(tensors):
            self._pack[1].run()
            if getattr(self, "rnn", None) is not None:
                self.rnn.refresh_weights(state_dict)
            return
        batch32 = (not self.hl8 and not self.hoist and os.environ.get("SSM_PACK_BATCH", "1") != "0"
                   and all(t.is_cuda and t.dtype == torch.float32 and t.is_contiguous() for t in tensors))
        if batch32 and getattr(self, "_pack32", None) is not None and self._pack32[0] == hb.PackBatch.key(tensors):
            self._pack32[1].run()
            if "final_conv" in self.layers:
                self.final_wb = (state_dict[param_key("final_conv", "weight")].detach(), state_dict[param_key("final_conv", "bias")].detach())
            if getattr(self, "rnn", None) is not None:
                self.rnn.refresh_weights(state_dict)
            return
        for name, (ci, co, k) in self.layers.items():
            w = state_dict[param_key(name, "weight")].to(device=self.device, dtype=torch.float32)
            b = state_dict[param_key(name, "bias")].to(device=self.device, dtype=torch.float32)
            if check_shapes:
                assert tuple(w.shape) == (co, ci, k, k), "%s: weight shape %s != %s" % (name, tuple(w.shape), (co, ci, k, k))
            s = layer_scale(name)
            if name == "final_conv":
                self.final_wb = (w.contiguous(), b.contiguous())
            if self.hl8:
                self.pk[name] = hb.PackedConv16(w, b, self.W // s, q8=self.q8, ups=self.fuse_up and name in self.UPS,
                                                scale=self.scales.get(name))
                self.scales.setdefault(name, self.pk[name].scale)
            else:
                nb = self.Bd if name in self.DECODER else self.B
                ups = self.fuse_up and name in self.UPS
                algo_args = (name, ci, co, k, nb, self.H // s, self.W // s, ups, self.wino, self.wino1d, self.wino4, self.blocked2d)
                cls = _ALGO_CLASS[choose_algo(*algo_args)]()
                pair_cls = cls
                if cls is hb.PackedUpGemm:
                    pair_cls = _ALGO_CLASS[choose_algo(*algo_args, upgemm=False)]()
                    batch32 = False
                if self.hoist and name == "conv1a":
                    zb = torch.zeros_like(b)
                    self.pk[name] = cls(w[:, 3:13].contiguous(), b, nb, self.H // s, self.W // s)
                    self.pk_pair[name] = cls(torch.cat([w[:, 13:16], w[:, 0:3]], 1).contiguous(), zb, self.hoist[0], self.H // s, self.W // s)
                elif self.hoist and name == "conv7a" and self.cross:
                    zb = torch.zeros_like(b)
                    self.pk[name] = cls(w[:, :512].contiguous(), b, nb, self.H // s, self.W // s, ups=ups)
                    self.pk_pair[name] = pair_cls(w[:, 512:].contiguous(), zb, self.hoist[0], self.H // s, self.W // s, ups=ups)
                elif (ups and cls is hb.PackedWino4 and name in WINO4_SUBPIXEL and not self.twins
                      and hb.subpixel_wino4_supported(ci, co, self.H // s, self.W // s)):
                    self.pk[name] = hb.PackedSubpixelWino4(w, b, nb, self.H // s, self.W // s)
                    batch32 = False
                else:
                    self.pk[name] = cls(w, b, nb, self.H // s, self.W // s, pool=name in POOLED, ups=ups)
        for pkk in list(self.pk.values()) + list(getattr(self, "pk_pair", {}).values()):
            if self.wino and isinstance(pkk, hb.PackedConv):
                pkk.split_ok = True
        ug = [(pkk, name) for name, pkk in self.pk.items() if isinstance(pkk, hb.PackedUpGemm)]
        if ug:
            need = max(pkk.scratch_floats(self.Bd, self.H // layer_scale(name), self.W // layer_scale(name)) for pkk, name in ug)
            if getattr(self, "_upgemm_scratch", None) is None or self._upgemm_scratch.numel() < need:
                self._upgemm_scratch = torch.empty(need, dtype=torch.float32, device=self.device)
            for pkk, _ in ug:
                pkk.scratch = self._upgemm_scratch
        self._pack32 = None
        if batch32:
            entries = [(self.pk[name], state_dict[param_key(name, "weight")], state_dict[param_key(name, "bias")], False)
                       for name in self.layers]
            self._pack32 = (hb.PackBatch.key(tensors), hb.PackBatch32(entries, self.device))
        self._pack = None
        if batchable:
            entries = [(self.pk[name], state_dict[param_key(name, "weight")], state_dict[param_key(name, "bias")], False)
                       for name in self.layers]
            self._pack = (hb.PackBatch.key(tensors), hb.PackBatch(entries, self.device))
        if getattr(self, "rnn", None) is not None:
            self.rnn.refresh_weights(state_dict)

    def _v(self, name, **kw):
        if self._b0 and name in self.ENCODER_T:
            kw["b0"] = self._b0
        return self.t[name].view(**kw)

    def _conv(self, name, src, dst, pool=None, src2=None, lrelu=True):
        pk = self.pk[name]
        s = self.t[src]
        d = self.t[dst]
        c2 = self.t[src2].C if src2 else 0
        tm = self.timer
        if tm is not None:
            fl = 2.0 * self._Bcur * s.H * s.W * pk.cout * pk.cin * pk.k * pk.k
            e0, e1 = tm.span("conv", "s%d.%s" % (self.stage, name), fl, issued=fl * issued_factor(pk))
            e0.record()
        v = self._v
        if self.hl8:
            final = name == "final_conv"
            y32 = v(dst) if final else (self.f32[dst].view() if self.twins else None)
            hb.conv2d_hl8(v(src), s.G * 8, v(src2) if src2 else None, c2, pk, None if final else v(dst),
                          y32, v(pool) if pool else None, self._Bcur, s.H, s.W,
                          lrelu=lrelu, fast=self.mode == "f16" or ("s%d.%s" % (self.stage, name)) in UNetPlan.fast_layers)
        elif self.hoist and name == "conv1a":
            assert self._pair_parts_ready, "hoisted stage-2 plan: run_pair_parts() must run before the per-t launches of a pass"
            conv_fn(pk)(v(src, c0=3), 10, None, 0, pk, v(dst), None, self._Bcur, s.H, s.W, lrelu=lrelu, add=self.t["pair1a"].view(), add_div=self.hoist[1])
        else:
            conv_fn(pk)(v(src), s.C, v(src2) if src2 else None, c2, pk, v(dst), v(pool) if pool else None, self._Bcur, s.H, s.W, lrelu=lrelu)
        if tm is not None:
            e1.record()

    def _bview(self, b, b_planes, b_broadcast, b_b0):
        if b_planes is not None:
            return b_planes, b_planes.view(broadcast=b_broadcast, b0=b_b0)
        if b:
            return self.t[b], self._v(b)
        return None, None

    SUBPIXEL = tuple(n for n in os.environ.get("SSM_SUBPIXEL", "conv11a,conv10a").split(",") if n not in ("", "0"))

    def _subpixel(self, name, a, b):
        if name not in self.SUBPIXEL or not self.q8 or self.twins or b is None:
            return None
        if name not in self.sp:
            from .subpixel import SubpixelUpConv
            A, Bp = self.t[a], self.t[b]
            wt = self._sd_for_sp[param_key(name, "weight")]
            assert wt.shape[1] == A.C + Bp.C == 8 * (A.G + Bp.G), "sub-pixel form expects whole channel groups"
            self.sp[name] = SubpixelUpConv(wt, self._sd_for_sp[param_key(name, "bias")], A.G, Bp.G, self.Bd, A.H, A.W, self.device)
        return self.sp[name]

    def _up_conv(self, name, a, b, u, dst, b_planes=None, b_broadcast=False, b_b0=0):
        if not self.fuse_up:
            self._up(a, b, u, b_planes=b_planes, b_broadcast=b_broadcast, b_b0=b_b0)
            return self._conv(name, u, dst)
        sp = self._subpixel(name, a, b) if b_planes is None else None
        if sp is not None:
            tm = self.timer
            if tm is not None:
                d, pk0 = self.t[dst], self.pk[name]
                e0, e1 = tm.span("conv", "s%d.%s" % (self.stage, name), 2.0 * self._Bcur * d.H * d.W * pk0.cout * pk0.cin * 9)
                e0.record()
            sp.run(lambda y0, x0: self._v(a, y0=y0, x0=x0), lambda y0, x0: self._v(b, y0=y0, x0=x0), self.t[dst])
            if tm is not None:
                e1.record()
            return
        pk = self.pk[name]
        A = self.t[a]
        Bp, bview = self._bview(b, b_planes, b_broadcast, b_b0)
        d = self.t[dst]
        tm = self.timer
        if tm is not None:
            fl = 2.0 * self._Bcur * d.H * d.W * pk.cout * pk.cin * 9
            e0, e1 = tm.span("conv", "s%d.%s" % (self.stage, name), fl, issued=fl * issued_factor(pk))
            e0.record()
        if self.hl8:
            hb.conv2d_ups_hl8(self._v(a), A.G * 8, bview, Bp.G * 8 if Bp else 0, pk,
                              d.view(), self.f32[dst].view() if self.twins else None, self._Bcur, d.H, d.W, lrelu=True,
                              fast=self.mode == "f16" or ("s%d.%s" % (self.stage, name)) in UNetPlan.fast_layers)
        elif isinstance(pk, hb.PackedSubpixelWino4) and b_planes is None:
            hb.conv2d_ups_subpixel_wino4(lambda y0, x0: self._v(a, y0=y0, x0=x0), A.C, (lambda y0, x0: self._v(b, y0=y0, x0=x0)) if b else None,
                                         Bp.C if Bp else 0, pk, lambda y0, x0: d.view(y0=y0, x0=x0), self._Bcur, d.H, d.W, lrelu=True)
        elif self.hoist and name == "conv7a" and self.cross:
            assert self._pair_parts_ready, "hoisted stage-2 plan: run_pair_parts() must run before the per-t launches of a pass"
            conv_fn(pk, True)(self._v(a), A.C, None, 0, pk, d.view(), self._Bcur, d.H, d.W, lrelu=True, add=self.t["pair7a"].view(), add_div=self.hoist[1])
        else:
            conv_fn(pk, True)(self._v(a), A.C, bview, Bp.C if Bp else 0, pk, d.view(), self._Bcur, d.H, d.W, lrelu=True)
        if tm is not None:
            e1.record()

    def _up(self, a, b, dst, b_planes=None, b_broadcast=False, b_b0=0):
        lib = hb.load()
        A = self.t[a]
        Bp, bview = self._bview(b, b_planes, b_broadcast, b_b0)
        tm = self.timer
        if tm is not None:
            e0, e1 = tm.span("upsample_cat", "s%d.%s" % (self.stage, dst),
                             nbytes=4.0 * self._Bcur * A.H * A.W * (A.C + (Bp.C if Bp else 0)) * 5)
            e0.record()
        if self.hl8:
            hb.check(lib.ssm_upsample2x_cat_hl8_fwd(self._v(a), A.G, bview if Bp else hb.NULL_HVIEW,
                                                    Bp.G if Bp else 0, self.t[dst].view(), self._Bcur, A.H, A.W,
                                                    hb.stream_ptr()))
        else:
            hb.check(lib.ssm_upsample2x_cat_fwd(self._v(a), A.C, bview if Bp else hb.NULL_VIEW,
                                                Bp.C if Bp else 0, self.t[dst].view(), self._Bcur, A.H, A.W,
                                                hb.stream_ptr()))
        if tm is not None:
            e1.record()

    def run_pair_parts(self, pair_planes, c6_planes):
        B1 = self.hoist[0]
        self._pair_parts_ready = True
        tm = self.timer
        pk = self.pk_pair["conv1a"]
        P = self.t["pair1a"]
        if tm is not None:
            fl = 2.0 * B1 * P.H * P.W * pk.cout * pk.cin * pk.k * pk.k
            e0, e1 = tm.span("conv", "s2.conv1a(pair)", fl, issued=fl * issued_factor(pk))
            e0.record()
        conv_fn(pk)(pair_planes.view(), 6, None, 0, pk, P.view(), None, B1, P.H, P.W, lrelu=False)
        if tm is not None:
            e1.record()
        if self.cross:
            pk = self.pk_pair["conv7a"]
            P = self.t["pair7a"]
            if tm is not None:
                fl = 2.0 * B1 * P.H * P.W * pk.cout * pk.cin * 9
                e0, e1 = tm.span("conv", "s2.conv7a(pair)", fl, issued=fl * issued_factor(pk))
                e0.record()
            conv_fn(pk, True)(c6_planes.view(), 512, None, 0, pk, P.view(), B1, P.H, P.W, lrelu=False)
            if tm is not None:
                e1.record()

    def run(self, cross_planes=None, cross_broadcast=False, cross_b0=0, synth=None):
        self.run_encoder()
        self.run_bottleneck()
        return self.run_decoder(cross_planes, cross_broadcast, cross_b0, synth)

    def run_encoder(self):
        c = self._conv
        self._b0, self._Bcur = 0, self.B
        c("conv1a", "in", "t1a")
        c("conv1b", "t1a", "c1", pool="p2")
        c("conv2a", "p2", "t2a")
        c("conv2b", "t2a", "c2", pool="p3")
        c("conv3a", "p3", "t3a")
        c("conv3b", "t3a", "c3", pool="p4")
        c("conv4a", "p4", "t4a")
        c("conv4b", "t4a", "c4", pool="p5")
        c("conv5a", "p5", "t5a")
        c("conv5b", "t5a", "c5", pool="p6")

    def run_family(self, k):
        c = self._conv
        self._b0, self._Bcur = 0, self.B
        self._pair_parts_ready = self.hoist is not None
        if k == 7:
            c("conv1a", "in", "t1a")
            c("conv1b", "t1a", "c1", pool="p2")
        elif k == 5:
            c("conv2a", "p2", "t2a")
            c("conv2b", "t2a", "c2", pool="p3")
        else:
            assert self.rnn is None and (self.hoist or not self.cross) and self.dec_b0 == 0 and self.Bd == self.B
            for a, src, dst, pool in (("conv3a", "p3", "t3a", None), ("conv3b", "t3a", "c3", "p4"), ("conv4a", "p4", "t4a", None),
                                      ("conv4b", "t4a", "c4", "p5"), ("conv5a", "p5", "t5a", None), ("conv5b", "t5a", "c5", "p6")):
                c(a, src, dst, pool=pool)
            self.run_bottleneck()
            self._decode(c, self._up_conv, None, False, 0, final=False)

    def run_bottleneck(self):
        self._b0, self._Bcur = 0, self.B
        if self.rnn is not None:
            tm = self.timer
            if tm is not None:
                e0, e1 = tm.span("conv", "s%d.conv6(%s)" % (self.stage, self.bottleneck), self.rnn.flops())
                e0.record()
            self.rnn.run(self.t["p6"], self.t["c6"])
            if tm is not None:
                e1.record()
            return
        self._conv("conv6.0", "p6", "t6a")
        self._conv("conv6.1", "t6a", "c6")

    def run_decoder(self, cross_planes=None, cross_broadcast=False, cross_b0=0, synth=None):
        c, uc = self._conv, self._up_conv
        self._b0, self._Bcur = self.dec_b0, self.Bd
        try:
            return self._decode(c, uc, cross_planes, cross_broadcast, cross_b0, synth)
        finally:
            self._b0, self._Bcur = 0, self.B
            self._pair_parts_ready = False

    def _final(self, synth):
        if not self.final4:
            assert synth is None
            self._conv("final_conv", "tf", "out", lrelu=False)
            return self.t["out"]
        tf, out = self.t["tf"], self.t["out"]
        w, b = self.final_wb
        tm = self.timer
        if tm is not None:
            e0, e1 = tm.span("conv", "s%d.final_conv" % self.stage, 2.0 * self._Bcur * tf.H * tf.W * out.C * tf.C * 9)
            e0.record()
        if synth is not None:
            synth(tf, w, b)
        else:
            nv = hb.NULL_VIEW
            hb.check(hb.load().ssm_final_conv_fwd(tf.view(), w.data_ptr(), b.data_ptr(), out.C, out.view(), nv, nv, None, nv, nv,
                                                  self._Bcur, tf.H, tf.W, hb.stream_ptr()))
        if tm is not None:
            e1.record()
        return None if synth is not None else out

    def _decode(self, c, uc, cross_planes, cross_broadcast, cross_b0, synth=None, final=True):
        if self.cross:
            if cross_planes is None and not self.hoist:
                raise RuntimeError("stage 2 was built with CROSS_SKIP but no stage-1 encoding was given")
            uc("conv7a", "c6", None, "u7", "t7a", b_planes=cross_planes, b_broadcast=cross_broadcast, b_b0=cross_b0)
        else:
            uc("conv7a", "c6", None, "u7", "t7a")
        c("conv7b", "t7a", "c7")
        uc("conv8a", "c7", "c5", "u8", "t8a")
        c("conv8b", "t8a", "c8")
        uc("conv9a", "c8", "c4", "u9", "t9a")
        c("conv9b", "t9a", "c9")
        uc("conv10a", "c9", "c3", "u10", "t10a")
        c("conv10b", "t10a", "c10")
        uc("conv11a", "c10", "c2", "u11", "t11a")
        c("conv11b", "t11a", "c11")
        c("fuse_conv", "c11", "tf", src2="c1")
        return self._final(synth) if final else None


# ... 477 lines not shown
```

superslomo-videointerpolation-pytorch_amd/ssm_amd/hipbind.py:

```python
import ctypes
import os
import threading

import torch

_HERE = os.path.dirname(os.path.abspath(__file__))
LIB_PATH = os.environ.get("SSM_HIP_LIB") or os.path.join(os.path.dirname(_HERE), "lib", "libssm_hip.so")

SSM_PADX = 4
SSM_PADY = 3
SSM_TAIL_SLACK_FLOATS = 1 << 16
SSM_LIGHT_ROW = 9
SSM_HDR_ROW = 8
SSM_HDR_PQ, SSM_HDR_HLG = 0, 1
SSM_ACC_WEIGHTS_MAX = 64
SSM_FLAG_LRELU = 1
SSM_FLAG_MASK = 8


class SsmView(ctypes.Structure):
    _fields_ = [("ptr", ctypes.c_void_p), ("sb", ctypes.c_longlong), ("sc", ctypes.c_longlong),
                ("sh", ctypes.c_int)]


NULL_VIEW = SsmView(None, 0, 0, 0)


class SsmHView(ctypes.Structure):
    _fields_ = [("ptr", ctypes.c_void_p), ("sb", ctypes.c_longlong), ("sg", ctypes.c_longlong),
                ("sp", ctypes.c_longlong), ("sh", ctypes.c_int)]


NULL_HVIEW = SsmHView(None, 0, 0, 0, 0)
SSM_FLAG_FP16_FAST = 2
SSM_FLAG_Q8 = 4

_c_int, _c_float, _vp, _sz = ctypes.c_int, ctypes.c_float, ctypes.c_void_p, ctypes.c_size_t
_ip = ctypes.POINTER(ctypes.c_int)

SIGNATURES = {
    "ssm_abi_version": (_c_int, []),
    "ssm_last_error_string": (ctypes.c_char_p, []),
    "ssm_plane_dims": (None, [_c_int, _c_int, _ip, _ip]),
    "ssm_copy_view": (_c_int, [SsmView, SsmView, _c_int, _c_int, _c_int, _c_int, _vp]),
    "ssm_conv_config": (_c_int, [_c_int, _c_int, _c_int, _c_int, _c_int, _c_int, _ip, _ip]),
    "ssm_packed_weight_floats": (_sz, [_c_int, _c_int, _c_int, _c_int]),
    "ssm_packed_bias_floats": (_sz, [_c_int, _c_int]),
    "ssm_pack_weights": (_c_int, [_vp, _vp, _vp, _vp, _c_int, _c_int, _c_int, _c_int, _c_int, _vp]),
    "ssm_conv2d_fwd": (_c_int, [SsmView, _c_int, SsmView, _c_int, _vp, _vp, SsmView, SsmView, _c_int, _c_int,
                                _c_int, _c_int, _c_int, _c_float, _c_int, _vp]),
    "ssm_conv2d_add_fwd": (_c_int, [SsmView, _c_int, SsmView, _c_int, _vp, _vp, SsmView, SsmView, SsmView, _c_int, _c_int, _c_int,
                                    _c_int, _c_int, _c_int, _c_float, _c_int, _vp]),
    "ssm_conv2d_ups_add_fwd": (_c_int, [SsmView, _c_int, SsmView, _c_int, _vp, _vp, SsmView, SsmView, _c_int, _c_int, _c_int, _c_int,
                                        _c_int, _c_float, _c_int, _vp]),
    "ssm_wino_conv2d_add_fwd": (_c_int, [SsmView, _c_int, SsmView, _c_int, _vp, _vp, SsmView, SsmView, SsmView, _c_int, _c_int, _c_int,
                                         _c_int, _c_int, _c_float, _c_int, _vp]),
    "ssm_wino_conv2d_ups_add_fwd": (_c_int, [SsmView, _c_int, SsmView, _c_int, _vp, _vp, SsmView, SsmView, _c_int, _c_int, _c_int, _c_int,
                                             _c_int, _c_float, _c_int, _vp]),
    "ssm_wino_plan": (_c_int, [_c_int, _c_int, _c_int, _c_int, _c_int, _c_int, _ip, _ip, _ip]),
    "ssm_wino_splitk_plan": (_c_int, [_c_int, _c_int, _c_int, _c_int, _c_int, _c_int, _c_int, _ip]),
    "ssm_conv_splitk_plan": (_c_int, [_c_int, _c_int, _c_int, _c_int, _c_int, _c_int, _ip]),
    "ssm_conv2d_splitk_fwd": (_c_int, [SsmView, _c_int, SsmView, _c_int, _vp, _vp, SsmView, _c_int, _c_int, _c_int, _c_int, _c_int, _c_int, _vp]),
    "ssm_wino_conv2d_splitk_fwd": (_c_int, [SsmView, _c_int, SsmView, _c_int, _vp, _vp, SsmView, _c_int, _c_int, _c_int, _c_int, _c_int, _c_int,
                                            _c_int, _vp]),
    "ssm_splitk_finish_fwd": (_c_int, [SsmView, _c_int, SsmView, SsmView, SsmView, _c_int, _c_int, _c_int, _c_int, _c_int, _c_float, _c_int, _vp]),
    "ssm_wino_force_kind": (_c_int, [_c_int]),
    "ssm_wino_packed_weight_floats": (_sz, [_c_int, _c_int, _c_int]),
    "ssm_wino_pack_weights": (_c_int, [_vp, _vp, _vp, _vp, _c_int, _c_int, _c_int, _vp]),
    "ssm_pack32_weights_batch": (_c_int, [_vp, _c_int, ctypes.c_longlong, _vp]),
    "ssm_pack32_wino_tiles_batch": (_c_int, [_vp, _c_int, ctypes.c_longlong, _c_int, _vp]),
    "ssm_wino4_plan": (_c_int, [_c_int, _c_int, _c_int, _c_int, _c_int, _c_int, _ip, _ip, _ip]),
    "ssm_wino4_force_kind": (_c_int, [_c_int]),
    "ssm_wino4_preferred": (_c_int, [_c_int, _c_int, _c_int, _c_int, _c_int, _c_int]),
    "ssm_wino_estimate": (ctypes.c_double, [_c_int, _c_int, _c_int, _c_int, _c_int, _c_int]),
    "ssm_wino4_packed_weight_floats": (_sz, [_c_int, _c_int]),
    "ssm_wino4_pack_weights": (_c_int, [_vp, _vp, _vp, _vp, _c_int, _c_int, _vp]),
    "ssm_wino4_conv2d_add_fwd": (_c_int, [SsmView, _c_int, SsmView, _c_int, _vp, _vp, SsmView, SsmView, SsmView, _c_int, _c_int, _c_int,
                                          _c_int, _c_int, _c_float, _c_int, _vp]),
    "ssm_wino4_conv2d_ups_add_fwd": (_c_int, [SsmView, _c_int, SsmView, _c_int, _vp, _vp, SsmView, SsmView, _c_int, _c_int, _c_int, _c_int,
                                              _c_int, _c_float, _c_int, _vp]),
    "ssm_upgemm_supported": (_c_int, [_c_int, _c_int, _c_int, _c_int, _c_int]),
    "ssm_upgemm_preferred": (_c_int, [_c_int, _c_int, _c_int, _c_int, _c_int]),
    "ssm_upgemm_force_kind": (_c_int, [_c_int]),
    "ssm_upgemm_packed_weight_floats": (_sz, [_c_int, _c_int]),
    "ssm_upgemm_pack_weights": (_c_int, [_vp, _vp, _c_int, _c_int, _vp]),
    "ssm_upgemm_scratch_floats": (_sz, [_c_int, _c_int, _c_int, _c_int]),
    "ssm_upgemm_conv2d_ups_add_fwd": (_c_int, [SsmView, _c_int, SsmView, _c_int, _vp, _vp, SsmView, SsmView, SsmView, _c_int, _c_int, _c_int,
                                               _c_int, _c_int, _c_float, _c_int, _vp]),
    "ssm_wino4_conv2d_shuffle_fwd": (_c_int, [SsmView, _c_int, SsmView, _c_int, _vp, _vp, SsmView, _c_int, _c_int, _c_int, _c_int, _c_float, _c_int, _vp]),
    "ssm_wino4_conv2d_ups_border_fwd": (_c_int, [SsmView, _c_int, SsmView, _c_int, _vp, _vp, SsmView, _c_int, _c_int, _c_int, _c_int, _c_float, _c_int,
                                                 _vp]),
    "ssm_wino1d_plan": (_c_int, [_c_int, _c_int, _c_int, _c_int, _c_int, _c_int, _ip, _ip, _ip]),
    "ssm_wino1d_force_kind": (_c_int, [_c_int]),
    "ssm_wino1d_packed_weight_floats": (_sz, [_c_int, _c_int, _c_int, _c_int]),
    "ssm_wino1d_pack_weights": (_c_int, [_vp, _vp, _vp, _vp, _c_int, _c_int, _c_int, _c_int, _c_int, _vp]),
    "ssm_wino1d_conv2d_add_fwd": (_c_int, [SsmView, _c_int, _vp, _vp, SsmView, SsmView, SsmView, _c_int, _c_int, _c_int, _c_int, _c_int,
                                           _c_int, _c_float, _c_int, _vp]),
    "ssm_wino5_plan": (_c_int, [_c_int, _c_int, _c_int, _c_int, _c_int, _ip]),
    "ssm_wino5_force_kind": (_c_int, [_c_int]),
    "ssm_wino5_packed_weight_floats": (_sz, [_c_int, _c_int]),
    "ssm_wino5_pack_weights": (_c_int, [_vp, _vp, _vp, _vp, _c_int, _c_int, _c_int, _vp]),
    "ssm_wino5_conv2d_add_fwd": (_c_int, [SsmView, _c_int, _vp, _vp, SsmView, SsmView, SsmView, _c_int, _c_int, _c_int, _c_int, _c_int,
                                          _c_float, _c_int, _vp]),
    "ssm_wino7_plan": (_c_int, [_c_int, _c_int, _c_int, _c_int, _c_int, _ip]),
    "ssm_wino7_force_kind": (_c_int, [_c_int]),
    "ssm_wino7_packed_weight_floats": (_sz, [_c_int, _c_int]),
    "ssm_wino7_pack_weights": (_c_int, [_vp, _vp, _vp, _vp, _c_int, _c_int, _vp]),
    "ssm_wino7_conv2d_add_fwd": (_c_int, [SsmView, _c_int, _vp, _vp, SsmView, SsmView, SsmView, _c_int, _c_int, _c_int, _c_int, _c_int,
                                          _c_float, _c_int, _vp]),
    "ssm_wino_conv2d_fwd": (_c_int, [SsmView, _c_int, SsmView, _c_int, _vp, _vp, SsmView, SsmView, _c_int, _c_int, _c_int, _c_int,
                                     _c_float, _c_int, _vp]),
    "ssm_wino_conv2d_ups_fwd": (_c_int, [SsmView, _c_int, SsmView, _c_int, _vp, _vp, SsmView, _c_int, _c_int, _c_int, _c_int,
                                         _c_float, _c_int, _vp]),
    "ssm_conv16_config": (_c_int, [_c_int, _c_int, _c_int, _ip, _ip]),
    "ssm_conv16_plan": (_c_int, [_c_int, _c_int, _c_int, _c_int, _c_int, _c_int, _ip, _ip, _ip]),
    "ssm_packed16_weight_halves": (_sz, [_c_int, _c_int, _c_int, _c_int]),
    "ssm_pack16_weights": (_c_int, [_vp, _vp, _vp, _vp, _c_int, _c_int, _c_int, _c_int, _c_int, _c_int, _c_float, _vp]),
    "ssm_conv2d_hl8_fwd": (_c_int, [SsmHView, _c_int, SsmHView, _c_int, _vp, _vp, _c_float, SsmHView, SsmView, SsmHView,
                                    _c_int, _c_int, _c_int, _c_int, _c_int, _c_float, _c_int, _vp]),
    "ssm_conv16q_config": (_c_int, [_c_int, _c_int, _c_int, _ip, _ip]),
    "ssm_conv16q_ups_config": (_c_int, [_c_int, _c_int, _ip, _ip]),
    "ssm_packed16q_weight_bytes": (_sz, [_c_int, _c_int, _c_int, _c_int, _c_int]),
    "ssm_pack16q_weights": (_c_int, [_vp, _vp, _vp, _vp, _c_int, _c_int, _c_int, _c_int, _c_int, _c_int, _c_float, _vp]),
    "ssm_hq8_from_f32": (_c_int, [SsmView, SsmHView, _c_int, _c_int, _c_int, _c_int, _c_int, _vp]),
    "ssm_hq8_to_f32": (_c_int, [SsmHView, SsmView, _c_int, _c_int, _c_int, _c_int, _c_int, _vp]),
    "ssm_conv16_ups_config": (_c_int, [_c_int, _c_int, _ip, _ip]),
    "ssm_conv2d_ups_hl8_fwd": (_c_int, [SsmHView, _c_int, SsmHView, _c_int, _vp, _vp, _c_float, SsmHView, SsmView,
                                        _c_int, _c_int, _c_int, _c_int, _c_float, _c_int, _vp]),
    "ssm_hl8_from_f32": (_c_int, [SsmView, SsmHView, _c_int, _c_int, _c_int, _c_int, _c_int, _vp]),
    "ssm_hl8_to_f32": (_c_int, [SsmHView, SsmView, _c_int, _c_int, _c_int, _c_int, _c_int, _vp]),
    "ssm_upsample2x_cat_hl8_fwd": (_c_int, [SsmHView, _c_int, SsmHView, _c_int, SsmHView, _c_int, _c_int, _c_int, _vp]),
    "ssm_flowinterp_inputs_hl8_fwd": (_c_int, [SsmView, SsmView, _vp, SsmHView, SsmView, _c_int, _c_int, _c_int, _vp]),
    "ssm_flowinterp_inputs_hq8_fwd": (_c_int, [SsmView, SsmView, _vp, SsmHView, SsmView, _c_int, _c_int, _c_int, _vp]),
    "ssm_frames_from_u8_fwd": (_c_int, [_vp, SsmView, _c_int, _c_int, _c_int, _c_int, _c_int, _c_int, _c_int,
                                        ctypes.POINTER(_c_float), ctypes.POINTER(_c_float), _c_int, _vp]),
    "ssm_frames_to_u8_fwd": (_c_int, [SsmView, _vp, _c_int, _c_int, _c_int, _c_int, _c_int, ctypes.POINTER(_c_float),
                                      ctypes.POINTER(_c_float), _c_int, _vp]),
    "ssm_frames_from_yuv_fwd": (_c_int, [_vp, SsmView, _c_int, _c_int, _c_int, _c_int, _c_int, _c_int, _c_int,
                                         ctypes.POINTER(_c_float), ctypes.POINTER(_c_float), _c_int, ctypes.POINTER(_c_float), _c_int,
                                         _c_int, _c_int, _vp]),
    "ssm_frames_to_yuv_fwd": (_c_int, [SsmView, _vp, _c_int, _c_int, _c_int, _c_int, _c_int, ctypes.POINTER(_c_float),
                                       ctypes.POINTER(_c_float), ctypes.POINTER(_c_float), _c_int, _c_int, _c_int, _vp]),
    "ssm_frames_from_yuvx_fwd": (_c_int, [_vp, SsmView, _c_int, _c_int, _c_int, _c_int, _c_int, _c_int, _c_int,
                                          ctypes.POINTER(_c_float), ctypes.POINTER(_c_float), _c_int, ctypes.POINTER(_c_float), _c_int,
                                          _c_int, _c_int, _c_int, _vp]),
    "ssm_frames_to_yuvx_fwd": (_c_int, [SsmView, _vp, _c_int, _c_int, _c_int, _c_int, _c_int, ctypes.POINTER(_c_float),
                                        ctypes.POINTER(_c_float), ctypes.POINTER(_c_float), _c_int, _c_int, _c_int, _c_int, _vp]),
    "ssm_clip_batch_from_u8_fwd": (_c_int, [_vp, ctypes.c_longlong, _vp, _vp, _vp, _vp, _c_int, _c_int, _c_int, _c_int, _c_int,
                                            ctypes.POINTER(_c_float), ctypes.POINTER(_c_float), _vp]),
    "ssm_frame_metrics_workspace_bytes": (_sz, [_c_int, _c_int, _c_int]),
    "ssm_frame_metrics_fwd": (_c_int, [_vp, _vp, _c_int, _c_int, _c_int, _vp, _sz, _vp, _vp]),
    "ssm_flow_metrics_workspace_bytes": (_sz, [_c_int, _c_int, _c_int]),
    "ssm_flow_metrics_fwd": (_c_int, [SsmView, _vp, _c_int, _c_int, _c_int, _c_int, _c_int, _c_int, _vp, _sz, _vp, _vp]),
    "ssm_flow_to_rgb_workspace_bytes": (_sz, [_c_int, _c_int, _c_int]),
    "ssm_flow_to_rgb_fwd": (_c_int, [SsmView, _vp, _c_int, _c_int, _c_int, _c_int, _c_int, _vp, _sz, _vp]),
    "ssm_warp_bilinear_bwd": (_c_int, [SsmView, SsmView, SsmView, SsmView, SsmView, _c_int, _c_int, _c_int, _c_int, _vp]),
    "ssm_lrelu_bwd": (_c_int, [SsmView, SsmView, SsmView, SsmView, _c_int, _c_int, _c_int, _c_int, _c_float, _c_int, _vp]),
    "ssm_lrelu_bwd_q8": (_c_int, [SsmView, SsmView, SsmView, SsmView, SsmHView, _c_int, _c_int, _c_int, _c_int, _c_float, _c_int, _vp]),
    "ssm_bias_grad": (_c_int, [SsmView, _vp, _c_int, _c_int, _c_int, _c_int, _vp]),
    "ssm_conv2d_wgrad_bias": (_c_int, [SsmView, SsmView, _vp, _vp, _c_int, _c_int, _c_int, _c_int, _c_int, _c_int, _c_int, _c_int, _c_int, _vp]),
    "ssm_conv_plan": (_c_int, [_c_int] * 8 + [ctypes.POINTER(ctypes.c_int)] * 3),
    "ssm_conv_force_kind": (_c_int, [_c_int]),
    "ssm_conv2d_ups_fwd": (_c_int, [SsmView, _c_int, SsmView, _c_int, _vp, _vp, SsmView, _c_int, _c_int, _c_int, _c_int, ctypes.c_float,
                                    _c_int, _vp]),
    "ssm_conv2d_hl8_subpixel_fwd": (_c_int, [SsmHView, _c_int, SsmHView, _c_int, _vp, _vp, ctypes.c_float, SsmHView, _c_int, _c_int, _c_int,
                                              _c_int, _c_int, _c_float, _c_int, _vp]),
    "ssm_hl8_gather_cols": (_c_int, [SsmHView, _c_int, SsmHView, _c_int, SsmHView, _c_int, _c_int, _c_int, _c_int, _c_int, _vp]),
    "ssm_conv16_subpixel_table_bytes": (ctypes.c_size_t, [_c_int]),
    "ssm_conv16_subpixel_plan": (_c_int, [_vp, _c_int, _c_int, _c_int, _c_int, ctypes.c_float, _c_int, _vp, ctypes.c_size_t,
                                          ctypes.POINTER(ctypes.c_int)]),
    "ssm_conv16_subpixel_run": (_c_int, [_vp, _c_int, ctypes.POINTER(ctypes.c_int), _c_int, _c_int, _c_int, _vp]),
    "ssm_pack16q_job_blocks": (_c_int, [_c_int, _c_int, _c_int, _c_int, ctypes.POINTER(ctypes.c_int), ctypes.POINTER(ctypes.c_int)]),
    "ssm_pack16q_weights_batch": (_c_int, [_vp, _c_int, _c_int, _vp]),
    "ssm_bias_grad_acc": (_c_int, [SsmView, _vp, _c_int, _c_int, _c_int, _c_int, _vp]),
    "ssm_conv2d_wgrad": (_c_int, [SsmView, SsmView, _vp, _c_int, _c_int, _c_int, _c_int, _c_int, _c_int, _c_int, _c_int, _c_int, _vp]),
    "ssm_conv2d_wgrad_bf16x3": (_c_int, [SsmView, SsmView, _vp, _c_int, _c_int, _c_int, _c_int, _c_int, _c_int, _c_int, _c_int, _c_int, _vp]),
    "ssm_splitk_enable": (_c_int, [_c_int, _c_int]),
    "ssm_program_create": (_c_int, [ctypes.POINTER(_vp)]),
    "ssm_program_destroy": (_c_int, [_vp]),
    "ssm_program_begin": (_c_int, [_vp, ctypes.POINTER(_vp), _c_int]),
    "ssm_program_mark": (_c_int, [_vp, ctypes.POINTER(_c_int)]),
    "ssm_program_end": (_c_int, [_vp, ctypes.POINTER(_c_int)]),
    "ssm_program_run": (_c_int, [_vp, _c_int, _c_int, ctypes.POINTER(_vp), _c_int]),
    "ssm_stream_wait": (_c_int, [_vp, _vp]),
    "ssm_wgrad_wino_supported": (_c_int, [_c_int] * 5),
    "ssm_wgrad_wino_scratch_floats": (ctypes.c_longlong, [_c_int, _c_int]),
    "ssm_conv2d_wgrad_wino": (_c_int, [SsmView, SsmView, _vp, _vp, _c_int, _c_int, _c_int, _c_int, _c_int, _c_int, _c_int, _vp]),
    "ssm_wgrad_wino_finish": (_c_int, [_vp, _c_int, _c_int, _c_float, _vp]),
    "ssm_upsample2x_cat_bwd": (_c_int, [SsmView, SsmView, _c_int, SsmView, _c_int, _c_int, _c_int, _c_int, _c_int, _c_int, _vp]),
    "ssm_upsample2x_cat_bwd_mask": (_c_int, [SsmView, SsmView, _c_int, SsmView, _c_int, SsmView, _c_float, _c_int, _c_int, _c_int, _c_int, _c_int, _vp]),
    "ssm_synthesize_bwd": (_c_int, [SsmView, SsmView, SsmView, SsmView, _vp, _vp, _vp, SsmView, SsmView, SsmView, _c_int, _c_int,
                                    _c_int, _c_int, _vp]),
    "ssm_maxpool2_fwd": (_c_int, [SsmView, SsmView, _c_int, _c_int, _c_int, _c_int, _vp]),
    "ssm_maxpool2_bwd": (_c_int, [SsmView, SsmView, SsmView, _c_int, _c_int, _c_int, _c_int, _vp]),
    "ssm_sqdiff_grad": (_c_int, [SsmView, SsmView, _vp, SsmView, _c_int, _c_int, _c_int, _c_int, _vp]),
    "ssm_sqdiff_mean": (_c_int, [SsmView, SsmView, _vp, _vp, _c_int, _c_int, _c_int, _c_int, _vp]),
    "ssm_train_loss_sums": (_c_int, [SsmView, SsmView, SsmView, SsmView, SsmView, SsmView, _vp, _vp, _c_int, _c_int, _c_int, _c_int, _c_int, _vp]),
    "ssm_flowinterp_inputs_bwd": (_c_int, [SsmView, SsmView, SsmView, SsmView, _vp, _vp, SsmView, _c_int, _c_int, _c_int, _c_int,
                                           _vp]),
    "ssm_convlstm_cell_fwd": (_c_int, [SsmView, SsmView, SsmView, SsmView, SsmView, SsmHView, _c_int, _c_int, _c_int, _c_int, _c_int, _vp]),
    "ssm_convgru_reset_fwd": (_c_int, [SsmView, SsmView, SsmView, SsmView, SsmHView, _c_int, _c_int, _c_int, _c_int, _c_int, _vp]),
    "ssm_convgru_update_fwd": (_c_int, [SsmView, SsmView, SsmView, SsmView, SsmView, SsmView, SsmHView, _c_int, _c_int, _c_int,
                                        _c_int, _c_int, _vp]),
    "ssm_convlstm_cell_bwd": (_c_int, [SsmView] * 7 + [_c_int, _c_int, _c_int, _c_int, _vp]),
    "ssm_convgru_reset_bwd": (_c_int, [SsmView] * 5 + [_c_int, _c_int, _c_int, _c_int, _vp]),
    "ssm_convgru_update_bwd": (_c_int, [SsmView] * 7 + [_c_int, _c_int, _c_int, _c_int, _vp]),
    "ssm_avgpool2_fwd": (_c_int, [SsmView, SsmView, _c_int, _c_int, _c_int, _c_int, _vp]),
    "ssm_upsample2x_cat_fwd": (_c_int, [SsmView, _c_int, SsmView, _c_int, SsmView, _c_int, _c_int, _c_int, _vp]),
    "ssm_warp_bilinear_fwd": (_c_int, [SsmView, SsmView, SsmView, _c_int, _c_int, _c_int, _c_int, _vp]),
    "ssm_flowinterp_inputs_fwd": (_c_int, [SsmView, SsmView, _vp, SsmView, _c_int, _c_int, _c_int, _vp]),
    "ssm_final_conv_fwd": (_c_int, [SsmView, _vp, _vp, _c_int, SsmView, SsmView, SsmView, _vp, SsmView, SsmView, _c_int, _c_int, _c_int, _vp]),
    "ssm_flowinterp_inputs_t_fwd": (_c_int, [SsmView, SsmView, _vp, SsmView, _c_int, _c_int, _c_int, _vp]),
    "ssm_synthesize_fwd": (_c_int, [SsmView, SsmView, SsmView, _vp, SsmView, SsmView, _c_int, _c_int, _c_int, _vp]),
    "ssm_synthesize_upscaled_fwd": (_c_int, [SsmView, SsmView, _vp, SsmView, _c_int, _c_int, _c_int, _c_int, _vp]),
    "ssm_tile_stitch_fwd": (_c_int, [SsmView, SsmView] + [_c_int] * 14 + [_vp]),
    "ssm_frames_accumulate_fwd": (_c_int, [SsmView, SsmView, _c_int, _c_int, _c_int, _c_int, _c_int, _c_float, _vp]),
    "ssm_frames_accumulate_light_fwd": (_c_int, [SsmView, SsmView, _c_int, _c_int, _c_int, _c_int, _c_float, _vp, _vp, _vp, _c_int, _vp]),
    "ssm_frames_accumulate_hdr_fwd": (_c_int, [SsmView, SsmView, _c_int, _c_int, _c_int, _c_int, _c_float, _vp, _vp, _c_int, _vp, _c_int, _vp]),
    "ssm_frames_accumulate_weighted_fwd": (_c_int, [SsmView, SsmView, _c_int, _c_int, _c_int, _c_int, _c_int, _c_float, _vp, _vp]),
    "ssm_frames_accumulate_light_weighted_fwd": (_c_int, [SsmView, SsmView, _c_int, _c_int, _c_int, _c_int, _c_float, _vp, _vp, _vp, _vp, _c_int,
                                                          _vp]),
    "ssm_frames_accumulate_hdr_weighted_fwd": (_c_int, [SsmView, SsmView, _c_int, _c_int, _c_int, _c_int, _c_float, _vp, _vp, _vp, _c_int, _vp,
                                                        _c_int, _vp]),
    "ssm_luma_sad_fwd": (_c_int, [_vp, _vp, ctypes.c_longlong, ctypes.c_longlong, _c_int, _c_int, _c_int, _vp, _vp]),
    "ssm_field_diff_fwd": (_c_int, [_vp, _vp, ctypes.c_longlong, ctypes.c_longlong, _c_int, _c_int, _c_int, _c_int, _vp, _vp]),
    "ssm_field_order_sums_fwd": (_c_int, [_vp, _vp, _vp, ctypes.c_longlong, ctypes.c_longlong, ctypes.c_longlong, _c_int, _c_int, _c_int, _c_int, _vp,
                                          _vp]),
    "ssm_plane_sse_fwd": (_c_int, [_vp, _vp, ctypes.c_longlong, ctypes.c_longlong, _c_int, _c_int, _c_int, _c_int, _c_int, _vp, _vp]),
    "ssm_block_sad_fwd": (_c_int, [_vp, _vp, ctypes.c_longlong, ctypes.c_longlong, _c_int, _c_int, _c_int, _c_int, _c_int, _c_int, _vp, _vp]),
    "ssm_static_paste_fwd": (_c_int, [_vp, _vp, ctypes.c_longlong, ctypes.c_longlong, _vp, ctypes.c_longlong, _c_int, _c_int, _c_int, _c_int,
                                      _c_int, _c_int, ctypes.c_uint, _vp, _vp]),
    "ssm_plane_ssim_fwd": (_c_int, [_vp, _vp, ctypes.c_longlong, ctypes.c_longlong, _c_int, _c_int, _c_int, _c_int, _c_int, ctypes.c_longlong,
                                    ctypes.c_longlong, _vp, _vp]),
    "ssm_payload_mix_fwd": (_c_int, [_vp, _vp, ctypes.c_longlong, ctypes.c_longlong, _vp, ctypes.c_longlong, _c_int, ctypes.c_longlong, _c_int,
                                     _c_int, _c_int, _c_int, _vp]),
    "ssm_fields_split_fwd": (_c_int, [_vp, _vp, _c_int, _c_int, _c_int, _c_int, _c_int, _vp]),
    "ssm_fields_weave_fwd": (_c_int, [_vp, ctypes.c_longlong, _vp, ctypes.c_longlong, _vp, ctypes.c_longlong, _c_int, _c_int, _c_int, _c_int,
                                      _c_int, _c_int, _c_int, _vp]),
    "ssm_luma_counts_fwd": (_c_int, [_vp, ctypes.c_longlong, _c_int, _c_int, _c_int, _c_int, _c_int, _vp, _vp, _vp]),
    "ssm_window_cut_fwd": (_c_int, [_vp, ctypes.c_longlong, _vp, ctypes.c_longlong] + [_c_int] * 9 + [_vp]),
}

_lib = None

# ... 308 lines not shown
                   lib.ssm_pack_weights, self.cout, self.cin, self.cin_p, self.k, self.bn)


def conv2d(x1, c1, x2, c2, pk, y, pool, B, H, W, lrelu=True, slope=0.1, add=None, add_div=1):
    lib = load()
    assert pk.cin_p == c1 + c2, "packed filter expects %d input channels, got %d" % (pk.cin_p, c1 + c2)
    assert (pk.bn, pk.ck) == conv_plan(pk.k, c1 + c2, pk.cout, B, H, W, pool is not None)[1:], \
        "filter was packed for another tile configuration (batch/size/pool changed)"
    if pool is None and x2 is None and c2 == 0 and getattr(pk, "split_ok", False):
        key = (B, H, W)
        cache = pk.__dict__.setdefault("_splitk", {})
        if key not in cache:
            ks = ctypes.c_int(1)
            check(lib.ssm_conv_splitk_plan(pk.k, c1 + c2, pk.cout, B, H, W, ctypes.byref(ks)))
            cache[key] = ks.value
        ks = cache[key]
        if ks > 1:
            return _splitk_launch(lib.ssm_conv2d_splitk_fwd, (B, H, W, pk.cout, pk.k), x1, c1, None, 0, pk, y, None, add, add_div, ks, B, H, W,
                                  SSM_FLAG_LRELU if lrelu else 0, slope)
    check(lib.ssm_conv2d_add_fwd(x1, c1, x2 if x2 is not None else NULL_VIEW, c2, pk.w.data_ptr(), pk.b.data_ptr(), y,
                                 pool if pool is not None else NULL_VIEW, add if add is not None else NULL_VIEW, add_div, B, H, W,
                                 pk.cout, pk.k, slope, SSM_FLAG_LRELU if lrelu else 0, stream_ptr()))


def conv2d_ups(a, c1, b, c2, pk, y, B, H, W, lrelu=True, slope=0.1, add=None, add_div=1):
    lib = load()
    assert pk.k == 3 and pk.cin_p == c1 + c2, "packed 3x3 filter expects %d input channels, got %d" % (pk.cin_p, c1 + c2)
    assert (pk.bn, pk.ck) == conv_plan(3, c1 + c2, pk.cout, B, H, W, False, True)[1:], \
        "filter was packed for another tile configuration (batch/size changed, or not packed with ups=True)"
    check(lib.ssm_conv2d_ups_add_fwd(a, c1, b if b is not None else NULL_VIEW, c2, pk.w.data_ptr(), pk.b.data_ptr(), y,
                                     add if add is not None else NULL_VIEW, add_div, B, H, W, pk.cout, slope,
                                     SSM_FLAG_LRELU if lrelu else 0, stream_ptr()))


def wino_plan(cin, cout, B, H, W, ups=False):
    return _plan(load().ssm_wino_plan, cin, cout, B, H, W, 1 if ups else 0)


def wino_supported(cin, cout, H, W, k=3):
    return k == 3 and cin % 8 == 0


class PackedWino(_PackedFilter):

    algo = "wino"

    def __init__(self, weight, bias, B, H, W, pool=False, ups=False):
        self._shape(weight, bias, ups)
        assert self.k == 3 and weight.shape[3] == 3, "the Winograd form is for 3x3 filters"
        _, self.bn, self.ck = wino_plan(self.cin, self.cout, B, H, W, self.ups)
        assert self.cin % self.ck == 0, "Cin must be a multiple of %d" % self.ck
        self.cin_p = self.cin
        lib = load()
        self._fill(weight, bias, lib.ssm_wino_packed_weight_floats(self.cout, self.cin, self.bn), lib.ssm_packed_bias_floats(self.cout, self.bn),
                   lib.ssm_wino_pack_weights, self.cout, self.cin, self.bn)


def wino_splitk(pk, B, H, W, ups=False):
    key = (B, H, W, bool(ups))
    cache = pk.__dict__.setdefault("_splitk", {})
    if key not in cache:
        ks = ctypes.c_int(1)
        check(load().ssm_wino_splitk_plan(pk.cin, pk.cout, B, H, W, 1 if ups else 0, pk.bn, ctypes.byref(ks)))
        cache[key] = ks.value
    return cache[key]


def _flags(lrelu, mask, add):
    if mask:
        assert add is not None and not lrelu, "mask epilogue: a mask source and no activation"
        return SSM_FLAG_MASK
    return SSM_FLAG_LRELU if lrelu else 0


def _splitk_launch(fwd, dims, x1, c1, x2, c2, pk, y, pool, add, add_div, ks, B, H, W, flags, slope):
    lib, st = load(), stream_ptr()
    scratch = pk.__dict__.setdefault("_splitk_part", {})
    key = (getattr(st, "value", st), ks, B, H, W)
    if key not in scratch:
        scratch[key] = Planes(ks * B, pk.cout, H, W, pk.w.device)
    part = scratch[key]
    check(fwd(x1, c1, x2 if x2 is not None else NULL_VIEW, c2, pk.w.data_ptr(), pk.b.data_ptr(), part.view(), ks, *dims, st))
    check(lib.ssm_splitk_finish_fwd(part.view(), ks, y, pool if pool is not None else NULL_VIEW, add if add is not None else NULL_VIEW, add_div,
                                    B, pk.cout, H, W, slope, flags, st))


def conv2d_wino(x1, c1, x2, c2, pk, y, pool, B, H, W, lrelu=True, slope=0.1, add=None, add_div=1, mask=False):
    lib = load()
    assert pk.cin == c1 + c2, "packed filter expects %d input channels, got %d" % (pk.cin, c1 + c2)
    assert (pk.bn, pk.ck) == wino_plan(c1 + c2, pk.cout, B, H, W, False)[1:], "filter was packed for another tile configuration"
    ks = wino_splitk(pk, B, H, W, False)
    if ks > 1:
        return _splitk_launch(lib.ssm_wino_conv2d_splitk_fwd, (0, B, H, W, pk.cout, pk.bn), x1, c1, x2, c2, pk, y, pool, add, add_div, ks, B, H, W,
                              _flags(lrelu, mask, add), slope)
    check(lib.ssm_wino_conv2d_add_fwd(x1, c1, x2 if x2 is not None else NULL_VIEW, c2, pk.w.data_ptr(), pk.b.data_ptr(), y,
                                      pool if pool is not None else NULL_VIEW, add if add is not None else NULL_VIEW, add_div, B, H, W,
                                      pk.cout, slope, _flags(lrelu, mask, add), stream_ptr()))


def conv2d_ups_wino(a, c1, b, c2, pk, y, B, H, W, lrelu=True, slope=0.1, add=None, add_div=1):
    lib = load()
    assert pk.cin == c1 + c2, "packed filter expects %d input channels, got %d" % (pk.cin, c1 + c2)
    assert (pk.bn, pk.ck) == wino_plan(c1 + c2, pk.cout, B, H, W, True)[1:], "filter was packed for another tile configuration"
    ks = wino_splitk(pk, B, H, W, True)
    if ks > 1:
        return _splitk_launch(lib.ssm_wino_conv2d_splitk_fwd, (1, B, H, W, pk.cout, pk.bn), a, c1, b, c2, pk, y, None, add, add_div, ks, B, H, W,
                              SSM_FLAG_LRELU if lrelu else 0, slope)
    check(lib.ssm_wino_conv2d_ups_add_fwd(a, c1, b if b is not None else NULL_VIEW, c2, pk.w.data_ptr(), pk.b.data_ptr(), y,
                                          add if add is not None else NULL_VIEW, add_div, B, H, W, pk.cout, slope,
                                          SSM_FLAG_LRELU if lrelu else 0, stream_ptr()))


def wino4_plan(cin, cout, B, H, W, ups=False):
    return _plan(load().ssm_wino4_plan, cin, cout, B, H, W, 1 if ups else 0)


def wino4_supported(cin, cout, H, W, k=3):
    return k == 3 and cin % 4 == 0 and cout % 32 == 0


def wino4_preferred(cin, cout, B, H, W, ups=False):
    return bool(load().ssm_wino4_preferred(cin, cout, B, H, W, 1 if ups else 0))


class PackedWino4(_PackedFilter):

    algo = "wino4"

    def __init__(self, weight, bias, B, H, W, pool=False, ups=False):
        self._shape(weight, bias, ups)
        assert self.k == 3 and weight.shape[3] == 3, "F(4x4,3x3) is for 3x3 filters"
        _, self.bn, self.ck = wino4_plan(self.cin, self.cout, B, H, W, self.ups)
        self.cin_p = self.cin
        lib = load()
        self._fill(weight, bias, lib.ssm_wino4_packed_weight_floats(self.cout, self.cin), self.cout, lib.ssm_wino4_pack_weights, self.cout, self.cin)


def conv2d_wino4(x1, c1, x2, c2, pk, y, pool, B, H, W, lrelu=True, slope=0.1, add=None, add_div=1, mask=False):
    lib = load()
    assert pk.cin == c1 + c2, "packed filter expects %d input channels, got %d" % (pk.cin, c1 + c2)
    check(lib.ssm_wino4_conv2d_add_fwd(x1, c1, x2 if x2 is not None else NULL_VIEW, c2, pk.w.data_ptr(), pk.b.data_ptr(), y,
                                       pool if pool is not None else NULL_VIEW, add if add is not None else NULL_VIEW, add_div, B, H, W,
                                       pk.cout, slope, _flags(lrelu, mask, add), stream_ptr()))


def conv2d_ups_wino4(a, c1, b, c2, pk, y, B, H, W, lrelu=True, slope=0.1, add=None, add_div=1):
    lib = load()
    assert pk.cin == c1 + c2, "packed filter expects %d input channels, got %d" % (pk.cin, c1 + c2)
    check(lib.ssm_wino4_conv2d_ups_add_fwd(a, c1, b if b is not None else NULL_VIEW, c2, pk.w.data_ptr(), pk.b.data_ptr(), y,
                                           add if add is not None else NULL_VIEW, add_div, B, H, W, pk.cout, slope,
                                           SSM_FLAG_LRELU if lrelu else 0, stream_ptr()))


WINO4_BORDER_TH, WINO4_BORDER_TW = 16, 32


def subpixel_wino4_supported(cin, cout, H, W):
    ty, tx = H // WINO4_BORDER_TH, W // WINO4_BORDER_TW
    return (cin % 4 == 0 and cout % 32 == 0 and H % WINO4_BORDER_TH == 0 and W % WINO4_BORDER_TW == 0 and ty >= 4 and tx >= 4
            and ((ty - 2) * WINO4_BORDER_TH // 2) % 16 == 0 and ((tx - 2) * WINO4_BORDER_TW // 2) % 32 == 0)


class PackedSubpixelWino4:

    algo = "wino4"

    def __init__(self, weight, bias, B, H, W):
        from .subpixel import effective_filter
        self.cout, self.cin, self.k = weight.shape[0], weight.shape[1], 3
        assert subpixel_wino4_supported(self.cin, self.cout, H, W), "sub-pixel F(4x4,3x3): unsupported shape"
        self.border = PackedWino4(weight, bias, B, H, W, ups=True)
        e = effective_filter(weight.detach().to(torch.float32), "int", "int")
        e = e.view(4, self.cout, self.cin, 3, 3).permute(1, 0, 2, 3, 4).reshape(4 * self.cout, self.cin, 3, 3).contiguous()
        self.inner = PackedWino4(e, bias.detach().to(torch.float32).repeat_interleave(4).contiguous(), B, H // 2, W // 2)
        self.w, self.b = self.border.w, self.border.b
        self.ups, self.cin_p, self.bn, self.ck = True, self.cin, self.border.bn, self.border.ck


def conv2d_ups_subpixel_wino4(a_view, c1, b_view, c2, pk, y_view, B, H, W, lrelu=True, slope=0.1):
    lib = load()
    flags = SSM_FLAG_LRELU if lrelu else 0
    y0, x0 = WINO4_BORDER_TH // 2, WINO4_BORDER_TW // 2
    h, w = H // 2 - 2 * y0, W // 2 - 2 * x0
    check(lib.ssm_wino4_conv2d_shuffle_fwd(a_view(y0, x0), c1, b_view(y0, x0) if b_view is not None else NULL_VIEW, c2, pk.inner.w.data_ptr(),
                                           pk.inner.b.data_ptr(), y_view(2 * y0, 2 * x0), B, h, w, 4 * pk.cout, slope, flags, stream_ptr()))
    check(lib.ssm_wino4_conv2d_ups_border_fwd(a_view(0, 0), c1, b_view(0, 0) if b_view is not None else NULL_VIEW, c2, pk.border.w.data_ptr(),
                                              pk.border.b.data_ptr(), y_view(0, 0), B, H, W, pk.cout, slope, flags, stream_ptr()))


def upgemm_supported(cin, cout, H, W, k=3):
    return bool(load().ssm_upgemm_supported(cin, cout, H, W, k))


def upgemm_preferred(cin, cout, B, H, W):
    return bool(load().ssm_upgemm_preferred(cin, cout, B, H // 2, W // 2))


def upgemm_scratch_view(buf, cout, h, w):
    wr = (w + 3) // 4 * 4
    return SsmView(buf.data_ptr(), 9 * cout * h * wr, h * wr, wr)


class PackedUpGemm(_PackedFilter):

    algo = "upgemm"

    def __init__(self, weight, bias, B, H, W, pool=False, ups=True):
        self._shape(weight, bias, True)
        assert ups and not pool, "the low-res GEMM form is for the fused-upsample layers"
        if not upgemm_supported(self.cin, self.cout, H, W, self.k):
            raise RuntimeError("low-res GEMM form: unsupported layer (%d -> %d, k = %d, output %d x %d)" % (self.cin, self.cout, self.k, H, W))
        self.cin_p, self.bn, self.ck = self.cin, 128, 16
        lib = load()
        self.w = torch.empty(lib.ssm_upgemm_packed_weight_floats(self.cout, self.cin), dtype=torch.float32, device=weight.device)
        self.b = bias.detach().contiguous().clone()
        check(lib.ssm_upgemm_pack_weights(weight.detach().contiguous().data_ptr(), self.w.data_ptr(), self.cout, self.cin, stream_ptr()))
        self.scratch = None

    def scratch_floats(self, B, H, W):
        return load().ssm_upgemm_scratch_floats(self.cout, B, H // 2, W // 2)


def conv2d_ups_upgemm(a, c1, b, c2, pk, y, B, H, W, lrelu=True, slope=0.1, add=None, add_div=1):
    lib = load()
    assert pk.cin == c1 + c2, "packed filter expects %d input channels, got %d" % (pk.cin, c1 + c2)
    need = pk.scratch_floats(B, H, W)
    if pk.scratch is None or pk.scratch.numel() < need:
        pk.scratch = torch.empty(need, dtype=torch.float32, device=pk.w.device)
    check(lib.ssm_upgemm_conv2d_ups_add_fwd(a, c1, b if b is not None else NULL_VIEW, c2, pk.w.data_ptr(), pk.b.data_ptr(),
                                            upgemm_scratch_view(pk.scratch, pk.cout, H // 2, W // 2), y,
                                            add if add is not None else NULL_VIEW, add_div, B, H, W, pk.cout, slope,
                                            SSM_FLAG_LRELU if lrelu else 0, stream_ptr()))


def wino1d_plan(k, cin, cout, B, H, W):
    return _plan(load().ssm_wino1d_plan, k, cin, cout, B, H, W)


def wino1d_supported(cin, cout, H, W, k):
    return k in (5, 7) and cout % 32 == 0


class PackedWino1d(_PackedFilter):

    algo = "wino1d"

    def __init__(self, weight, bias, B, H, W, pool=False, ups=False):
        self._shape(weight, bias, False)
        assert not ups, "the 7x7 / 5x5 layers have no fused-upsample form"
        assert self.k in (5, 7) and weight.shape[3] == self.k, "the 1-D Winograd form is for 7x7 and 5x5 filters"
        _, self.bn, self.ck = wino1d_plan(self.k, self.cin, self.cout, B, H, W)
        self.cin_p = (self.cin + self.ck - 1) // self.ck * self.ck
        lib = load()
        self._fill(weight, bias, lib.ssm_wino1d_packed_weight_floats(self.cout, self.cin_p, self.k, self.bn),
                   lib.ssm_packed_bias_floats(self.cout, self.bn), lib.ssm_wino1d_pack_weights, self.cout, self.cin, self.cin_p, self.k, self.bn)


def conv2d_wino1d(x1, c1, x2, c2, pk, y, pool, B, H, W, lrelu=True, slope=0.1, add=None, add_div=1):
    lib = load()
    assert x2 is None and c2 == 0, "the 1-D Winograd layers have no concatenated source"
    assert pk.cin_p == c1, "packed filter expects %d input channels, got %d" % (pk.cin_p, c1)
    assert (pk.bn, pk.ck) == wino1d_plan(pk.k, c1, pk.cout, B, H, W)[1:], "filter was packed for another tile configuration"
    check(lib.ssm_wino1d_conv2d_add_fwd(x1, c1, pk.w.data_ptr(), pk.b.data_ptr(), y, pool if pool is not None else NULL_VIEW,
                                        add if add is not None else NULL_VIEW, add_div, B, H, W, pk.cout, pk.k, slope,
                                        SSM_FLAG_LRELU if lrelu else 0, stream_ptr()))


def wino5_supported(cin, cout, H, W, k):
    return k == 5 and cout % 32 == 0


class PackedWino5(_PackedFilter):

    algo = "wino5"

    def __init__(self, weight, bias, B, H, W, pool=False, ups=False):
        self._shape(weight, bias, False)
        assert not ups, "the 5x5 layers have no fused-upsample form"
        assert self.k == 5 and weight.shape[3] == 5 and self.cout % 32 == 0, "the F(4x4,5x5) form is for 5x5 filters, Cout a multiple of 32"
        self.bn, self.ck = 32, 4
        self.cin_p = (self.cin + 3) // 4 * 4
        lib = load()
        self._fill(weight, bias, lib.ssm_wino5_packed_weight_floats(self.cout, self.cin_p), self.cout, lib.ssm_wino5_pack_weights,
                   self.cout, self.cin, self.cin_p)


def conv2d_wino5(x1, c1, x2, c2, pk, y, pool, B, H, W, lrelu=True, slope=0.1, add=None, add_div=1, mask=False):
    lib = load()
    assert x2 is None and c2 == 0, "the 5x5 layers have no concatenated source"
    assert pk.cin_p == c1, "packed filter expects %d input channels, got %d" % (pk.cin_p, c1)
    check(lib.ssm_wino5_conv2d_add_fwd(x1, c1, pk.w.data_ptr(), pk.b.data_ptr(), y, pool if pool is not None else NULL_VIEW,
                                       add if add is not None else NULL_VIEW, add_div, B, H, W, pk.cout, slope,
                                       _flags(lrelu, mask, add), stream_ptr()))


def wino7_supported(cin, cout, H, W, k):
    return k == 7 and cout % 32 == 0


class PackedWino7(_PackedFilter):

    algo = "wino7"

    def __init__(self, weight, bias, B, H, W, pool=False, ups=False):
        self._shape(weight, bias, False)
        assert not ups, "the 7x7 layers have no fused-upsample form"
        assert self.k == 7 and weight.shape[3] == 7, "the blocked Winograd form is for 7x7 filters"
        self.cout_p = (self.cout + 31) // 32 * 32
        self.bn, self.ck, self.cin_p = 32, 1, self.cin
        lib = load()
        self._fill(weight, bias, lib.ssm_wino7_packed_weight_floats(self.cout, self.cin), self.cout_p, lib.ssm_wino7_pack_weights,
                   self.cout, self.cin)


def conv2d_wino7(x1, c1, x2, c2, pk, y, pool, B, H, W, lrelu=True, slope=0.1, add=None, add_div=1):
    lib = load()
    assert x2 is None and c2 == 0, "the 7x7 layers have no concatenated source"
    assert pk.cin == c1, "packed filter expects %d input channels, got %d" % (pk.cin, c1)
    check(lib.ssm_wino7_conv2d_add_fwd(x1, c1, pk.w.data_ptr(), pk.b.data_ptr(), y, pool if pool is not None else NULL_VIEW,
                                       add if add is not None else NULL_VIEW, add_div, B, H, W, pk.cout_p, slope,
                                       SSM_FLAG_LRELU if lrelu else 0, stream_ptr()))


for _cls, _plain, _ups in ((PackedConv, conv2d, conv2d_ups), (PackedWino, conv2d_wino, conv2d_ups_wino),
                           (PackedWino4, conv2d_wino4, conv2d_ups_wino4), (PackedWino1d, conv2d_wino1d, None), (PackedWino5, conv2d_wino5, None),
                           (PackedWino7, conv2d_wino7, None), (PackedUpGemm, None, conv2d_ups_upgemm)):
    _cls.form = FORMS[_cls.algo]
    _cls.form.cls, _cls.form.launch, _cls.form.launch_ups = _cls, _plain, _ups


class HPlanes:

    def __init__(self, B, C, H, W, device, groups=None, q8=False):
        self.B, self.C, self.H, self.W = B, C, H, W
        self.q8 = bool(q8)
        self.G = groups if groups is not None else (C + 7) // 8
        if q8 and self.G % 2:
            self.G += 1
# ... 233 lines not shown
```

Baseline: 407.6.

## Share Winograd input transforms across cout blocks via global scratch

Adds a two-launch Winograd F(4x4,3x3) path for wide layers. The first launch handles a few cout blocks and also writes its transformed input tiles (V) to a global scratch buffer. The second launch covers the remaining cout blocks and DMA-reads V from scratch with a 3-buffer LDS pipeline instead of recomputing the input transform. This removes transform work that was repeated per cout block, at the cost of extra global memory traffic and scratch space, and splits the blocks between launches using a cost model of CU waves.

```diff
diff --git a/include/ssm_hip.h b/include/ssm_hip.h
--- a/include/ssm_hip.h
+++ b/include/ssm_hip.h
@@ -105,6 +105,15 @@
                                  int H, int W, int Cout4, float slope, int flags, void *stream);
 int ssm_wino4_conv2d_ups_border_fwd(ssm_view a, int C1, ssm_view b, int C2, const float *w_packed, const float *bias_packed, ssm_view y, int B,
                                     int H, int W, int Cout, float slope, int flags, void *stream);
+
+long long ssm_wino4_vshare_tiles(int Cin, int Cout, int B, int H, int W, int ups);
+long long ssm_wino4_vshare_scratch_floats(int Cin, int Cout, int B, int H, int W, int ups);
+int ssm_wino4_vshare_kw(long long tiles_batch, int nblocks);
+int ssm_wino4_vshare_preferred(int Cin, int Cout, int B, int H, int W, int ups);
+int ssm_wino4_vshare_set_mode(int mode);
+int ssm_wino4_vshare_fwd(int form, ssm_view x1, int C1, ssm_view x2, int C2, const float *w_packed, const float *bias_packed, ssm_view y,
+                         ssm_view pool, ssm_view add, int add_div, float *scratch, long long scratch_floats, int kw, int B, int H, int W, int Cout,
+                         float slope, int flags, void *stream);
 
 int ssm_upgemm_supported(int Cin, int Cout, int H, int W, int k);
 int ssm_upgemm_preferred(int Cin, int Cout, int B, int h, int w);
diff --git a/superslomo-videointerpolation-pytorch_amd/csrc/ssm_wino4.hip b/superslomo-videointerpolation-pytorch_amd/csrc/ssm_wino4.hip
--- a/superslomo-videointerpolation-pytorch_amd/csrc/ssm_wino4.hip
+++ b/superslomo-videointerpolation-pytorch_amd/csrc/ssm_wino4.hip
@@ -5,6 +5,7 @@
 #include <mutex>
 #include <type_traits>
 #include <cstdlib>
+#include <cstring>
 
 namespace {
 
@@ -37,6 +38,8 @@
     const float *add;
     long long asb, asc;
     int ash, adiv;
+    float *vsc;
+    int nb0;
 };
 
 template <int GTX_, int WTY_, int WTX_, int NCB_ = 1>
@@ -82,6 +85,17 @@
     static_assert(BYTES + (C::NCB == 2 ? 256 : 0) <= (C::NCB == 1 ? 80 : 160) * 1024, "LDS budget (two workgroups of 256 or one of 512 per CU; 64-cout form: + its biases)");
 };
 
+template <class C>
+struct W4LdsR {
+    static constexpr int NW = 4;
+    static constexpr int NGU = C::USZ / 256, NGV = C::VSZ / 256;
+    static constexpr int NIU = (NGU + NW - 1) / NW, NIV = (NGV + NW - 1) / NW, NI = NIU + NIV;
+    static constexpr int UOFF = 0, VOFF = 2 * C::USZ, NBUF = 3;
+    static constexpr int BYTES = (VOFF + NBUF * C::VSZ) * 4;
+    static_assert(C::NCB == 2 && C::USZ % 256 == 0 && C::VSZ % 256 == 0 && NGU % NW == 0, "whole 1-KiB DMA groups; every wave brings NIU filter pieces");
+    static_assert(BYTES + 256 <= 160 * 1024 && NI <= 18, "LDS budget (+ the biases); DMA issue slots of the matrix loop");
+};
+
 #define W4_PA 0.625
 #define W4_PB 1.6
 constexpr float kA = (float)W4_PA, kB = (float)W4_PB, kA2 = (float)(W4_PA * W4_PA), kB2 = (float)(W4_PB * W4_PB);
@@ -325,10 +339,22 @@
     }
 }
 
-template <class C, bool UPS, bool SHUF = false>
+template <class C, bool UPS, int VSRC>
+struct W4Sel {
+    static constexpr int VOFF = W4Lds<C, UPS>::VOFF, BYTES = W4Lds<C, UPS>::BYTES, NI = W4Lds<C, UPS>::NI;
+};
+template <class C, bool UPS>
+struct W4Sel<C, UPS, 2> {
+    static constexpr int VOFF = W4LdsR<C>::VOFF, BYTES = W4LdsR<C>::BYTES, NI = W4LdsR<C>::NI;
+};
+
+template <class C, bool UPS, bool SHUF = false, int VSRC = 0>
 __global__ __launch_bounds__(C::THREADS, 2) void wino4_kernel(const W4Params p) {
     extern __shared__ __attribute__((aligned(16))) float lds[];
     using L = W4Lds<C, UPS>;
+    using S = W4Sel<C, UPS, VSRC>;
+    static_assert(VSRC == 0 || C::NCB == 2, "a shared V is for the 64-cout form");
+    static_assert(VSRC != 2 || !UPS, "a reader has no patch to expand: instantiate it with UPS = false");
     constexpr int BN = C::BN, PH = C::PH, PW = C::PW, CK = C::CK, NT = C::NT, NW = C::NW, NCB = C::NCB;
 
     const int tid = threadIdx.x;
@@ -337,7 +363,8 @@
     const int cb = wid & 1, tg = (wid >> 1) & 1, blk = wid >> 2;
 
     int id = ssm_xcd_tile(blockIdx.x, gridDim.x);
-    const int nb = id % p.NB;
+    const int nbl = id % p.NB;
+    const int nb = VSRC == 0 ? nbl : nbl + p.nb0;
     id /= p.NB;
     int tx, ty, b;
     if (UPS && C::NCB == 1 && p.border) {
@@ -359,6 +386,7 @@
         b = id / p.tilesY;
     }
     const int x0 = tx * C::TW, y0 = ty * C::TH;
+    const float *vblk = VSRC == 0 ? nullptr : p.vsc + (((long long)b * p.tilesY + ty) * p.tilesX + tx) * (long long)(p.Cin / C::CK) * C::VSZ;
 
     const long long porg = UPS ? (long long)(y0 / 2 - 1) * p.sh + (x0 / 2 - 4) : (long long)(y0 - 1) * p.sh + (x0 - 4);
     const float *pbase1 = p.src1 + (long long)b * p.sb1 + porg;
@@ -432,7 +460,7 @@
     }
     float bv[4];
     if constexpr (NCB == 2) {
-        if (tid < BN) lds[L::BYTES / 4 + tid] = p.bias[nb * BN + tid];
+        if (tid < BN) lds[S::BYTES / 4 + tid] = p.bias[nb * BN + tid];
     } else {
 #pragma unroll
         for (int r = 0; r < 4; ++r) bv[r] = p.bias[nb * BN + blk * 32 + cb * 16 + 4 * q + r];
@@ -445,11 +473,11 @@
     const int tgx = (ttile & 15) % C::GTX, tgy = (ttile & 15) / C::GTX, tg2 = ttile >> 4;
     const int tTx = (tg2 % C::WTX) * C::GTX + tgx, tTy = (tg2 / C::WTX) * C::GTY + tgy;
     const int t_src = L::POFF + (UPS ? 0 : C::SHIFT) + (tcin * PH + 4 * tTy) * PW + 4 * tTx + 3 + (UPS ? C::SHIFT : 0);
-    const int t_dst = L::VOFF / 4 + (tcin * 9) * NT + ttile;
+    const int t_dst = S::VOFF / 4 + (tcin * 9) * NT + ttile;
 
     const f32x4 *lds4 = (const f32x4 *)lds;
     const int aBase = L::UOFF / 4 + blk * (C::USZ1 / 4) + q * (9 * 32) + cb * 16 + l15;
-    const int bBase = L::VOFF / 4 + q * (9 * NT) + tg * 16 + l15;
+    const int bBase = S::VOFF / 4 + q * (9 * NT) + tg * 16 + l15;
 
     int ex_r0 = 0, ex_r1 = 0, ex_dd = 0, ex_fl = 0;
     if constexpr (UPS) {
@@ -603,7 +631,7 @@
                     __builtin_amdgcn_sched_barrier(0);
                 }
                 if constexpr (NCB == 2) {
-                    if ((e == 1 || e == 3) && 2 * g + (e == 3) < L::NI) {
+                    if ((e == 1 || e == 3) && 2 * g + (e == 3) < S::NI) {
                         dma(2 * g + (e == 3));
                         __builtin_amdgcn_sched_barrier(0);
                     }
@@ -663,6 +691,63 @@
         if (ch + 1 < nchunks) chunk1(ch++, T{}, F{});
         chunk1(ch, F{}, F{});
 
+    } else if constexpr (VSRC == 2) {
+        using R = W4LdsR<C>;
+        using T = std::true_type;
+        using F = std::false_type;
+        auto issue_r = [&](int ch, int stage, int vb, int k) {
+            if (k < R::NIU) {
+                constexpr int G1 = C::USZ1 / 256;
+                const int g = R::NW * k + wid, gb = g / G1;
+                const float *base = wbase + ((long long)gb * p.Cin + ch * CK) * (9 * 32 * 4) + (g - gb * G1) * 256;
+                const unsigned m0v = __builtin_amdgcn_readfirstlane(lds0 + (unsigned)(R::UOFF + stage * C::USZ) * 4u + (unsigned)g * 1024u);
+                lds_dma16(base, uoff, m0v);
+            } else {
+                const int kk = k - R::NIU, g = R::NW * kk + wid;
+                if (R::NW * kk + R::NW - 1 < R::NGV || g < R::NGV) {
+                    const float *base = vblk + (long long)ch * C::VSZ + g * 256;
+                    const unsigned m0v = __builtin_amdgcn_readfirstlane(lds0 + (unsigned)(R::VOFF + vb * C::VSZ) * 4u + (unsigned)g * 1024u);
+                    lds_dma16(base, uoff, m0v);
+                }
+            }
+        };
+        if (wid < R::NW) {
+#pragma unroll
+            for (int k = 0; k < R::NI; ++k) issue_r(0, 0, 0, k);
+            if (nchunks > 1) {
+#pragma unroll
+                for (int k = R::NIU; k < R::NI; ++k) issue_r(1, 0, 1, k);
+            }
+        }
+        const bool v_full = wid < R::NGV - R::NW * (R::NIV - 1);
+        auto chunkr = [&](int ch, int vb, auto STEADY, auto ISSUER) __attribute__((always_inline)) {
+            constexpr bool steady = decltype(STEADY)::value, issuer = decltype(ISSUER)::value;
+            const bool m1 = steady || ch + 1 < nchunks, m2 = steady || ch + 2 < nchunks;
+            const int st = ch & 1, vb2 = vb == 0 ? 2 : vb - 1;
+            if constexpr (issuer) {
+                if (!m1) wait_vmcnt<0>();
+                else if (v_full) wait_vmcnt<R::NIV>();
+                else wait_vmcnt<R::NIV - 1>();
+            }
+            __syncthreads();
+            matrix(st, vb, [&](int g) {
+                if constexpr (issuer) {
+                    if (g < R::NIU) {
+                        if (m1) issue_r(ch + 1, st ^ 1, 0, g);
+                    } else {
+                        if (m2) issue_r(ch + 2, 0, vb2, g);
+                    }
+                }
+            }, [](int) {});
+        };
+        auto chunksr = [&](auto ISSUER) __attribute__((always_inline)) {
+            int ch = 0, vb = 0;
+            for (; ch + 2 < nchunks; ++ch, vb = vb == 2 ? 0 : vb + 1) chunkr(ch, vb, T{}, ISSUER);
+            for (; ch < nchunks; ++ch, vb = vb == 2 ? 0 : vb + 1) chunkr(ch, vb, F{}, ISSUER);
+        };
+        if (wid < R::NW) chunksr(T{});
+        else chunksr(F{});
+
     } else {
         using T = std::true_type;
         using F = std::false_type;
@@ -734,11 +819,23 @@
                 }
             }
         };
-        auto chunk = [&](int ch, auto STEADY, auto HH, auto HQ) __attribute__((always_inline)) {
+        auto vcopy = [&](int m, int st, const float *vdst) __attribute__((always_inline)) {
+            constexpr int NGV = C::VSZ / 256;
+            if (m >= 23 && m < 33) {
+                const int k = (m - 23) % 5, g = 4 * k + (wid - 4);
+                if (4 * k + 3 < NGV || g < NGV) {
+                    if (m < 28) r4[k] = lds4[S::VOFF / 4 + st * (C::VSZ / 4) + g * 64 + lane];
+                    else store_sbase(vdst, (unsigned)(g * 64 + lane) * 16u, r4[k]);
+                }
+            }
+        };
+        const float *vcur = vblk;
+        auto chunk = [&](int ch, auto STEADY, auto HH, auto HQ, auto VW) __attribute__((always_inline)) {
             constexpr bool steady = decltype(STEADY)::value;
+            constexpr bool vw = VSRC == 1 && decltype(VW)::value && decltype(HQ)::value == 1;
             const bool m1 = steady || ch + 1 < nchunks, m2 = steady || ch + 2 < nchunks, m3 = steady || ch + 3 < nchunks;
             const int st = ch & 1;
-            wait_vmcnt<0>();
+            if constexpr (!vw) wait_vmcnt<0>();
             if (!W4ABL(16) || ch == 0) __syncthreads();
             W4STAMP(0)
             W4TRACE(ch, 0)
@@ -757,7 +854,9 @@
                 if constexpr (decltype(HQ)::value == 1) {
                     if (m1 && !W4ABL(4)) tstep2(HH, m, tsrc, tdst);
                 }
+                if constexpr (vw) vcopy(m, st, vcur);
             });
+            if constexpr (vw) vcur += C::VSZ;
             W4STAMP(3)
             W4TRACE(ch, 2)
             if constexpr (UPS) {
@@ -766,20 +865,24 @@
             W4STAMP(1)
             W4TRACE(ch, 3)
         };
-        auto chunks = [&](auto HH, auto HQ) __attribute__((always_inline)) {
+        auto chunks = [&](auto HH, auto HQ, auto VW) __attribute__((always_inline)) {
             if constexpr (decltype(HQ)::value == 1) __builtin_amdgcn_s_setprio(1);
             int ch = 0;
-            for (; ch + 3 < nchunks; ++ch) chunk(ch, T{}, HH, HQ);
-            for (; ch < nchunks; ++ch) chunk(ch, F{}, HH, HQ);
+            for (; ch + 3 < nchunks; ++ch) chunk(ch, T{}, HH, HQ, VW);
+            for (; ch < nchunks; ++ch) chunk(ch, F{}, HH, HQ, VW);
         };
         using I0 = std::integral_constant<int, 0>;
         using I1 = std::integral_constant<int, 1>;
+        using VW = std::integral_constant<bool, VSRC == 1>;
+        const bool vwg = VSRC == 1 && nbl == 0;
         if (thh == 0) {
-            if (thq == 0) chunks(I0{}, I0{});
-            else chunks(I0{}, I1{});
+            if (thq == 0) chunks(I0{}, I0{}, F{});
+            else if (vwg) chunks(I0{}, I1{}, VW{});
+            else chunks(I0{}, I1{}, F{});
         } else {
-            if (thq == 0) chunks(I1{}, I0{});
-            else chunks(I1{}, I1{});
+            if (thq == 0) chunks(I1{}, I0{}, F{});
+            else if (vwg) chunks(I1{}, I1{}, VW{});
+            else chunks(I1{}, I1{}, F{});
         }
     }
 
@@ -788,7 +891,7 @@
 #endif
     {
         if constexpr (NCB == 2) {
-            const f32x4 b4 = *(const f32x4 *)(lds + L::BYTES / 4 + blk * 32 + cb * 16 + 4 * q);
+            const f32x4 b4 = *(const f32x4 *)(lds + S::BYTES / 4 + blk * 32 + cb * 16 + 4 * q);
             bv[0] = b4[0], bv[1] = b4[1], bv[2] = b4[2], bv[3] = b4[3];
         }
         const int gx = l15 % C::GTX, gy = l15 / C::GTX;
@@ -887,22 +990,22 @@
     return best;
 }
 
-template <class C, bool UPS, bool SHUF = false>
-int w4launch(W4Params &p, int B, hipStream_t st) {
+template <class C, bool UPS, bool SHUF = false, int VSRC = 0>
+int w4launch(W4Params &p, int B, hipStream_t st, int nblocks = 0) {
     p.tilesX = (p.W + C::TW - 1) / C::TW;
     p.tilesY = (p.H + C::TH - 1) / C::TH;
     if (p.Cout % C::BN) {
         ssm::set_error("wino4 conv: tile configuration of %d couts per workgroup, Cout = %d", C::BN, p.Cout);
         return SSM_E_UNSUPPORTED;
     }
-    p.NB = p.Cout / C::BN;
+    p.NB = VSRC == 0 ? p.Cout / C::BN : nblocks;
     if (p.border && (!UPS || p.tilesX < 2 || p.tilesY < 2)) {
         ssm::set_error("wino4 conv: a border-ring launch needs the fused-upsample form and at least 2 x 2 workgroup tiles (%d x %d)", p.tilesX, p.tilesY);
         return SSM_E_UNSUPPORTED;
     }
     const long long ntiles = p.border ? 2LL * p.tilesX + 2LL * (p.tilesY - 2) : (long long)p.tilesX * p.tilesY;
     const long long blocks = ntiles * p.NB * B;
-    int lds_bytes = W4Lds<C, UPS>::BYTES + (C::NCB == 2 ? C::BN * 4 : 0);
+    int lds_bytes = W4Sel<C, UPS, VSRC>::BYTES + (C::NCB == 2 ? C::BN * 4 : 0);
 #ifdef W4_TRACE
     lds_bytes += 4096;
 #endif
@@ -910,8 +1013,8 @@
     if (const char *e = getenv("SSM_WINO4_SOLO"))
         if (atoi(e) && lds_bytes < 100 * 1024) lds_bytes = 100 * 1024;
 #endif
-    return ssm::launch_tiles<wino4_kernel<C, UPS, SHUF>>("wino4 conv", UPS ? "ssm_wino4_conv2d_ups_fwd" : "ssm_wino4_conv2d_fwd", blocks, C::THREADS,
-                                                          lds_bytes, st, p);
+    return ssm::launch_tiles<wino4_kernel<C, UPS, SHUF, VSRC>>("wino4 conv", VSRC ? "ssm_wino4_vshare_fwd" : UPS ? "ssm_wino4_conv2d_ups_fwd" : "ssm_wino4_conv2d_fwd",
+                                                                blocks, C::THREADS, lds_bytes, st, p);
 }
 
 template <bool UPS>
@@ -996,6 +1099,8 @@
     p.ws = W / 2;
     p.abl = 0;
     p.border = 0;
+    p.vsc = nullptr;
+    p.nb0 = 0;
 #ifdef SSM_WINO_ABLATE
     if (const char *e = getenv("SSM_WINO4_ABL")) p.abl = atoi(e);
 #endif
@@ -1113,3 +1218,105 @@
     if (rf != SSM_OK) return rf;
     return w4dispatch<true>(kind, p, B, (hipStream_t)stream);
 }
+
+namespace {
+
+constexpr int kVsCus = 256;
+
+int vshare_kind(int Cin, int Cout, int B, int H, int W, int ups) {
+    const int kind = pick_w4kind(Cin, Cout, B, H, W, ups);
+    return kW4Info[kind].bn == 64 ? kind : (int)Y4A_;
+}
+
+long long vshare_tiles(int kind, int H, int W) {
+    return (long long)((W + kW4Info[kind].tw - 1) / kW4Info[kind].tw) * ((H + kW4Info[kind].th - 1) / kW4Info[kind].th);
+}
+
+int vshare_kw(long long tb, int nblocks, long long *cost = nullptr) {
+    int best = 0;
+    long long bc = 0;
+    for (int kw = 1; kw < nblocks; ++kw) {
+        const long long c = 100 * ((tb * kw + kVsCus - 1) / kVsCus) + 87 * ((tb * (nblocks - kw) + kVsCus - 1) / kVsCus);
+        if (!best || c < bc) best = kw, bc = c;
+    }
+    if (cost) *cost = bc;
+    return best;
+}
+
+std::atomic<int> g_vshare_mode{-1};
+
+int vshare_mode() {
+    int m = g_vshare_mode.load();
+    if (m < 0) {
+        const char *e = getenv("SSM_WINO4_VSHARE");
+        m = !e ? 1 : !strcmp(e, "force") ? 2 : atoi(e) ? 1 : 0;
+        g_vshare_mode.store(m);
+    }
+    return m;
+}
+
+template <class C>
+int vshare_launch(int mode, W4Params &p, int B, int kw, int nblocks, hipStream_t st) {
+    p.nb0 = 0;
+    const int rw = mode == 2 ? w4launch<C, false, true, 1>(p, B, st, kw) : w4launch<C, false, false, 1>(p, B, st, kw);
+    if (rw != SSM_OK) return rw;
+    p.nb0 = kw;
+    return mode == 2 ? w4launch<C, false, true, 2>(p, B, st, nblocks - kw) : w4launch<C, false, false, 2>(p, B, st, nblocks - kw);
+}
+
+}
+
+extern "C" int ssm_wino4_vshare_kw(long long tiles_batch, int nblocks) {
+    return tiles_batch > 0 && nblocks >= 2 ? vshare_kw(tiles_batch, nblocks) : 0;
+}
+
+extern "C" long long ssm_wino4_vshare_tiles(int Cin, int Cout, int B, int H, int W, int ups) {
+    if (Cin % 4 || Cout % 64 || Cin <= 0 || Cout < 128 || B <= 0 || H <= 0 || W <= 0 || ups) return 0;
+    return vshare_tiles(vshare_kind(Cin, Cout, B, H, W, ups), H, W);
+}
+
+extern "C" long long ssm_wino4_vshare_scratch_floats(int Cin, int Cout, int B, int H, int W, int ups) {
+    return ssm_wino4_vshare_tiles(Cin, Cout, B, H, W, ups) * B * (Cin / 4) * (long long)Y4A::VSZ;
+}
+
+extern "C" int ssm_wino4_vshare_preferred(int Cin, int Cout, int B, int H, int W, int ups) {
+    const long long tiles = ssm_wino4_vshare_tiles(Cin, Cout, B, H, W, ups);
+    const int mode = vshare_mode();
+    if (!tiles || !mode) return 0;
+    if (mode == 2) return 1;
+    return 0;
+}
+
+extern "C" int ssm_wino4_vshare_set_mode(int mode) {
+    g_vshare_mode.store(mode < 0 ? -1 : mode > 2 ? 2 : mode);
+    return SSM_OK;
+}
+
+extern "C" int ssm_wino4_vshare_fwd(int form, ssm_view x1, int C1, ssm_view x2, int C2, const float *w_packed, const float *bias_packed, ssm_view y,
+                                    ssm_view pool, ssm_view add, int add_div, float *scratch, long long scratch_floats, int kw, int B, int H, int W,
+                                    int Cout, float slope, int flags, void *stream) {
+    SSM_REQUIRE(form >= 0 && form <= 2, "wino4 vshare: form %d is none of 0 plain, 1 fused upsample, 2 sub-pixel", form);
+    SSM_REQUIRE(Cout >= 128 && Cout % 64 == 0, "wino4 vshare: Cout (%d) must be a multiple of 64 and at least 128 (two cout blocks share a V)", Cout);
+    SSM_REQUIRE(form != 1, "wino4 vshare: the fused-upsample form has no writer kernel (it spills registers); use ssm_wino4_conv2d_ups_add_fwd");
+    SSM_REQUIRE(form == 0 || !pool.ptr, "wino4 vshare: only the plain form has a fused pool");
+    SSM_REQUIRE(form != 2 || !add.ptr, "wino4 vshare: the sub-pixel form has no addend");
+    const int rc = ssm_wino4_plan(C1 + C2, Cout, B, H, W, form == 1, nullptr, nullptr, nullptr);
+    if (rc != SSM_OK) return rc;
+    W4Params p;
+    const int rf = w4fill(p, x1, C1, x2, C2, w_packed, bias_packed, y, pool, add, add_div, B, H, W, Cout, slope, flags, form == 1 ? W / 2 : W);
+    if (rf != SSM_OK) return rf;
+    const int nblocks = Cout / 64, kind = vshare_kind(C1 + C2, Cout, B, H, W, form == 1);
+    const long long tiles = vshare_tiles(kind, H, W);
+    if (kw == 0) kw = vshare_kw(tiles * B, nblocks);
+    SSM_REQUIRE(kw >= 1 && kw < nblocks, "wino4 vshare: a writer launch of %d of %d cout blocks leaves no reader", kw, nblocks);
+    const long long need = tiles * B * ((C1 + C2) / 4) * (long long)Y4A::VSZ;
+    SSM_REQUIRE(scratch && ssm::aligned16(scratch), "wino4 vshare: the V scratch must be a 16-byte aligned device tensor");
+    SSM_REQUIRE(scratch_floats >= need, "wino4 vshare: the V scratch holds %lld floats, the layer needs %lld", scratch_floats, need);
+    SSM_REQUIRE(need * 4 < (1LL << 40), "wino4 vshare: V scratch too large");
+    p.vsc = scratch;
+    switch (kind) {
+        case Y4A_: return vshare_launch<Y4A>(form, p, B, kw, nblocks, (hipStream_t)stream);
+        case Y4B_: return vshare_launch<Y4B>(form, p, B, kw, nblocks, (hipStream_t)stream);
+        default: return vshare_launch<Y4C>(form, p, B, kw, nblocks, (hipStream_t)stream);
+    }
+}
diff --git a/superslomo-videointerpolation-pytorch_amd/ssm_amd/engine.py b/superslomo-videointerpolation-pytorch_amd/ssm_amd/engine.py
--- a/superslomo-videointerpolation-pytorch_amd/ssm_amd/engine.py
+++ b/superslomo-videointerpolation-pytorch_amd/ssm_amd/engine.py
@@ -62,6 +62,9 @@
 
 
 UPGEMM = os.environ.get("SSM_UPGEMM", "1")
+
+
+VSHARE_MAX_BYTES = 1 << 30
 
 
 def upgemm_enabled(name):
@@ -284,6 +287,7 @@
                 self._upgemm_scratch = torch.empty(need, dtype=torch.float32, device=self.device)
             for pkk, _ in ug:
                 pkk.scratch = self._upgemm_scratch
+        self._plan_vshare()
         self._pack32 = None
         if batch32:
             entries = [(self.pk[name], state_dict[param_key(name, "weight")], state_dict[param_key(name, "bias")], False)
@@ -296,6 +300,31 @@
             self._pack = (hb.PackBatch.key(tensors), hb.PackBatch(entries, self.device))
         if getattr(self, "rnn", None) is not None:
             self.rnn.refresh_weights(state_dict)
+
+    def vshare_problem(self, name):
+        pk = self.pk.get(name)
+        if not (self.wino and self.fuse_up and not self.twins) or (self.hoist and name in ("conv1a", "conv7a")):
+            return None
+        s = layer_scale(name)
+        nb = self.Bd if name in self.DECODER else self.B
+        if isinstance(pk, hb.PackedSubpixelWino4):
+            return (pk.cin, 4 * pk.cout, nb, self.H // s // 2 - hb.WINO4_BORDER_TH, self.W // s // 2 - hb.WINO4_BORDER_TW)
+        if isinstance(pk, hb.PackedWino4) and not pk.ups:
+            return (pk.cin, pk.cout, nb, self.H // s, self.W // s)
+        return None
+
+    def _plan_vshare(self):
+        self.vshare = {}
+        for name in self.pk:
+            prob = self.vshare_problem(name)
+            if prob is not None and prob[1] >= 128 and prob[1] % 64 == 0 and hb.wino4_vshare_preferred(*prob):
+                need = hb.wino4_vshare_scratch_floats(*prob)
+                if 0 < 4 * need <= VSHARE_MAX_BYTES:
+                    self.vshare[name] = need
+        need = max(self.vshare.values(), default=0)
+        self.vshare_bytes = 4 * need
+        if need and (getattr(self, "_vshare_scratch", None) is None or self._vshare_scratch.numel() < need):
+            self._vshare_scratch = torch.empty(need, dtype=torch.float32, device=self.device)
 
     def _v(self, name, **kw):
         if self._b0 and name in self.ENCODER_T:
@@ -322,6 +351,9 @@
         elif self.hoist and name == "conv1a":
             assert self._pair_parts_ready, "hoisted stage-2 plan: run_pair_parts() must run before the per-t launches of a pass"
             conv_fn(pk)(v(src, c0=3), 10, None, 0, pk, v(dst), None, self._Bcur, s.H, s.W, lrelu=lrelu, add=self.t["pair1a"].view(), add_div=self.hoist[1])
+        elif name in self.vshare:
+            hb.conv2d_wino4_vshare(v(src), s.C, v(src2) if src2 else None, c2, pk, v(dst), v(pool) if pool else None, self._Bcur, s.H, s.W,
+                                   self._vshare_scratch, lrelu=lrelu)
         else:
             conv_fn(pk)(v(src), s.C, v(src2) if src2 else None, c2, pk, v(dst), v(pool) if pool else None, self._Bcur, s.H, s.W, lrelu=lrelu)
         if tm is not None:
@@ -377,7 +409,8 @@
                               fast=self.mode == "f16" or ("s%d.%s" % (self.stage, name)) in UNetPlan.fast_layers)
         elif isinstance(pk, hb.PackedSubpixelWino4) and b_planes is None:
             hb.conv2d_ups_subpixel_wino4(lambda y0, x0: self._v(a, y0=y0, x0=x0), A.C, (lambda y0, x0: self._v(b, y0=y0, x0=x0)) if b else None,
-                                         Bp.C if Bp else 0, pk, lambda y0, x0: d.view(y0=y0, x0=x0), self._Bcur, d.H, d.W, lrelu=True)
+                                         Bp.C if Bp else 0, pk, lambda y0, x0: d.view(y0=y0, x0=x0), self._Bcur, d.H, d.W, lrelu=True,
+                                         scratch=self._vshare_scratch if name in self.vshare else None)
         elif self.hoist and name == "conv7a" and self.cross:
             assert self._pair_parts_ready, "hoisted stage-2 plan: run_pair_parts() must run before the per-t launches of a pass"
             conv_fn(pk, True)(self._v(a), A.C, None, 0, pk, d.view(), self._Bcur, d.H, d.W, lrelu=True, add=self.t["pair7a"].view(), add_div=self.hoist[1])
diff --git a/superslomo-videointerpolation-pytorch_amd/ssm_amd/hipbind.py b/superslomo-videointerpolation-pytorch_amd/ssm_amd/hipbind.py
--- a/superslomo-videointerpolation-pytorch_amd/ssm_amd/hipbind.py
+++ b/superslomo-videointerpolation-pytorch_amd/ssm_amd/hipbind.py
@@ -90,6 +90,13 @@
     "ssm_wino4_conv2d_shuffle_fwd": (_c_int, [SsmView, _c_int, SsmView, _c_int, _vp, _vp, SsmView, _c_int, _c_int, _c_int, _c_int, _c_float, _c_int, _vp]),
     "ssm_wino4_conv2d_ups_border_fwd": (_c_int, [SsmView, _c_int, SsmView, _c_int, _vp, _vp, SsmView, _c_int, _c_int, _c_int, _c_int, _c_float, _c_int,
                                                  _vp]),
+    "ssm_wino4_vshare_tiles": (ctypes.c_longlong, [_c_int, _c_int, _c_int, _c_int, _c_int, _c_int]),
+    "ssm_wino4_vshare_scratch_floats": (ctypes.c_longlong, [_c_int, _c_int, _c_int, _c_int, _c_int, _c_int]),
+    "ssm_wino4_vshare_kw": (_c_int, [ctypes.c_longlong, _c_int]),
+    "ssm_wino4_vshare_preferred": (_c_int, [_c_int, _c_int, _c_int, _c_int, _c_int, _c_int]),
+    "ssm_wino4_vshare_set_mode": (_c_int, [_c_int]),
+    "ssm_wino4_vshare_fwd": (_c_int, [_c_int, SsmView, _c_int, SsmView, _c_int, _vp, _vp, SsmView, SsmView, SsmView, _c_int, _vp, ctypes.c_longlong,
+                                      _c_int, _c_int, _c_int, _c_int, _c_int, _c_float, _c_int, _vp]),
     "ssm_wino1d_plan": (_c_int, [_c_int, _c_int, _c_int, _c_int, _c_int, _c_int, _ip, _ip, _ip]),
     "ssm_wino1d_force_kind": (_c_int, [_c_int]),
     "ssm_wino1d_packed_weight_floats": (_sz, [_c_int, _c_int, _c_int, _c_int]),
@@ -704,6 +711,31 @@
                                            SSM_FLAG_LRELU if lrelu else 0, stream_ptr()))
 
 
+VSHARE_PLAIN, VSHARE_SUBPIXEL = 0, 2
+
+
+def wino4_vshare_scratch_floats(cin, cout, B, H, W):
+    return int(load().ssm_wino4_vshare_scratch_floats(cin, cout, B, H, W, 0))
+
+
+def wino4_vshare_kw(tiles_batch, nblocks):
+    return int(load().ssm_wino4_vshare_kw(tiles_batch, nblocks))
+
+
+def wino4_vshare_preferred(cin, cout, B, H, W):
+    return bool(load().ssm_wino4_vshare_preferred(cin, cout, B, H, W, 0))
+
+
+def conv2d_wino4_vshare(x1, c1, x2, c2, pk, y, pool, B, H, W, scratch, lrelu=True, slope=0.1, add=None, add_div=1, kw=0, form=VSHARE_PLAIN,
+                        cout=None):
+    lib = load()
+    assert pk.cin == c1 + c2, "packed filter expects %d input channels, got %d" % (pk.cin, c1 + c2)
+    check(lib.ssm_wino4_vshare_fwd(form, x1, c1, x2 if x2 is not None else NULL_VIEW, c2, pk.w.data_ptr(), pk.b.data_ptr(), y,
+                                   pool if pool is not None else NULL_VIEW, add if add is not None else NULL_VIEW, add_div,
+                                   scratch.data_ptr() if scratch is not None else None, scratch.numel() if scratch is not None else 0, kw, B, H, W,
+                                   pk.cout if cout is None else cout, slope, _flags(lrelu, False, add), stream_ptr()))
+
+
 WINO4_BORDER_TH, WINO4_BORDER_TW = 16, 32
 
 
@@ -729,13 +761,17 @@
         self.ups, self.cin_p, self.bn, self.ck = True, self.cin, self.border.bn, self.border.ck
 
 
-def conv2d_ups_subpixel_wino4(a_view, c1, b_view, c2, pk, y_view, B, H, W, lrelu=True, slope=0.1):
+def conv2d_ups_subpixel_wino4(a_view, c1, b_view, c2, pk, y_view, B, H, W, lrelu=True, slope=0.1, scratch=None):
     lib = load()
     flags = SSM_FLAG_LRELU if lrelu else 0
     y0, x0 = WINO4_BORDER_TH // 2, WINO4_BORDER_TW // 2
     h, w = H // 2 - 2 * y0, W // 2 - 2 * x0
-    check(lib.ssm_wino4_conv2d_shuffle_fwd(a_view(y0, x0), c1, b_view(y0, x0) if b_view is not None else NULL_VIEW, c2, pk.inner.w.data_ptr(),
-                                           pk.inner.b.data_ptr(), y_view(2 * y0, 2 * x0), B, h, w, 4 * pk.cout, slope, flags, stream_ptr()))
+    if scratch is not None:
+        conv2d_wino4_vshare(a_view(y0, x0), c1, b_view(y0, x0) if b_view is not None else None, c2, pk.inner, y_view(2 * y0, 2 * x0), None, B, h, w,
+                            scratch, lrelu=lrelu, slope=slope, form=VSHARE_SUBPIXEL, cout=4 * pk.cout)
+    else:
+        check(lib.ssm_wino4_conv2d_shuffle_fwd(a_view(y0, x0), c1, b_view(y0, x0) if b_view is not None else NULL_VIEW, c2, pk.inner.w.data_ptr(),
+                                               pk.inner.b.data_ptr(), y_view(2 * y0, 2 * x0), B, h, w, 4 * pk.cout, slope, flags, stream_ptr()))
     check(lib.ssm_wino4_conv2d_ups_border_fwd(a_view(0, 0), c1, b_view(0, 0) if b_view is not None else NULL_VIEW, c2, pk.border.w.data_ptr(),
                                               pk.border.b.data_ptr(), y_view(0, 0), B, H, W, pk.cout, slope, flags, stream_ptr()))
 
```

Result: no change. 409.2 (median of 6 runs) (+0.4%).
